# cvlab-yonsei/HVPR

Hardware: AMD Instinct MI355X
Metric: KITTI frames/sec/GPU (fwd, ~20k pts); VFE+scatter achieved HBM GB/s vs peak (higher is better)
Workload: dtype f32; 1 GPU; hvpr_car.yaml batch=1 forward-only, a1..a8 (on-GPU voxelize, pillar VFE, memory read-out + scatter, BEV backbone, head + decode, score top-k + rotated-BEV NMS); frames sharded over ranks, replicas only; global_batch=1, weights=deterministic synthetic (seed 0), BN stats randomised, cls bias -4.595

## Files before the change

hvpr_amd/_lib.py:

```python
import ctypes
import os

_HERE = os.path.dirname(os.path.abspath(__file__))
ABI_VERSION = 8
LIB_PATH = os.environ.get("HVPR_AMD_LIB", os.path.join(_HERE, "libhvpr_amd.so"))

_c = ctypes
_P = _c.c_void_p
_I = _c.c_int
_F = _c.c_float
_Z = _c.c_size_t
ALLREDUCE_FN = _c.CFUNCTYPE(_I, _P, _I, _P, _P)

SIGNATURES = {
    "hvpr_abi_version": (_I, []),
    "hvpr_status_string": (_c.c_char_p, [_I]),
    "hvpr_set_batchnorm_allreduce": (None, [_P, _P]),
    "hvpr_voxelize_workspace_bytes": (_Z, [_I, _I, _I, _I, _I]),
    "hvpr_voxelize_workspace_reset": (_I, [_P, _Z, _I, _I, _I, _I, _I, _P]),
    "hvpr_voxelize_workspace_status": (_I, [_P, _Z, _I, _I, _I, _I, _I, _P]),
    "hvpr_voxelize_f32": (_I, [_P, _I, _I, _I, _I, _P, _I, _F, _F, _F, _F, _F, _F, _I, _I, _I, _I, _I, _I,
                               _P, _P, _P, _P, _I, _P, _Z, _I, _I, _P]),
    "hvpr_pillar_vfe_fwd_f32": (_I, [_P, _P, _P, _I, _I, _P, _F, _F, _F, _F, _F, _F, _P, _P, _P, _P, _P, _P, _P, _P,
                                     _P, _P, _P, _P]),
    "hvpr_memory_bank_packed_floats": (_Z, [_I]),
    "hvpr_memory_bank_pack_f32": (_I, [_P, _I, _P, _P]),
    "hvpr_memory_readout_fwd_f32": (_I, [_P, _I, _P, _P, _P, _I, _I, _P, _P, _P]),
    "hvpr_scatter_workspace_bytes": (_Z, [_I, _I, _I]),
    "hvpr_memory_scatter_fwd_f32": (_I, [_P, _P, _P, _I, _P, _P, _P, _I, _I, _I, _I, _I, _P, _P, _P, _P, _Z, _P]),
    "hvpr_encode_fwd_f32": (_I, [_P, _I, _I, _I, _I, _P, _I, _F, _F, _F, _F, _F, _F, _I, _I, _I, _I, _I, _I, _F, _F, _F,
                                 _P, _P, _P, _P, _P, _P, _P, _P, _P, _P, _I, _I, _P, _P, _P, _P, _I, _P, _P, _P, _P, _P, _P,
                                 _P, _P, _Z, _I, _I, _I, _P]),
    "hvpr_scatter_bev_fwd_f32": (_I, [_P, _I, _P, _I, _P, _I, _P, _I, _P, _I, _I, _I, _P, _P, _P, _Z, _P]),
    "hvpr_spatial_gate_f32": (_I, [_P, _I, _I, _I, _I, _P, _F, _F, _F, _P, _P]),
    "hvpr_head_decode_f32": (_I, [_P, _I, _I, _I, _I, _I, _I, _I, _P, _P, _P, _F, _F, _F, _P, _P, _P, _P, _P]),
    "hvpr_score_topk_workspace_bytes": (_Z, [_I, _I]),
    "hvpr_score_topk_f32": (_I, [_P, _I, _I, _F, _I, _I, _P, _P, _P, _P, _Z, _P]),
    "hvpr_nms_workspace_bytes": (_Z, [_I]),
    "hvpr_nms_bev_f32": (_I, [_P, _I, _P, _P, _I, _F, _I, _I, _P, _P, _P, _Z, _P]),
    "hvpr_gather_predictions_f32": (_I, [_P, _I, _P, _P, _P, _I, _P, _P, _P, _P, _P]),
    "hvpr_boxes_pairwise_f32": (_I, [_P, _I, _P, _I, _I, _P, _P]),
    "hvpr_boxes_pairwise_ragged_f32": (_I, [_P, _P, _P, _P, _P, _I, _c.c_longlong, _P, _P]),
    "hvpr_kitti_overlaps_f64": (_I, [_P, _P, _P, _P, _P, _P, _I, _c.c_longlong, _I, _P, _P]),
    "hvpr_kitti_match_workspace_bytes": (_Z, [_I, _I, _I, _I]),
    "hvpr_kitti_match_f64": (_I, [_P, _P, _P, _P, _P, _P, _P, _P, _I, _c.c_longlong, _P, _I, _I, _P, _I, _P, _I, _P, _P, _I, _I,
                                  _P, _P, _P, _P, _P, _Z, _P]),
    "hvpr_recall_record_f32": (_I, [_P, _P, _I, _I, _P, _I, _I, _P, _I, _P, _P, _P]),
    "hvpr_prediction_annos_f32": (_I, [_P, _P, _P, _P, _I, _I, _P, _P, _I, _P, _c.c_longlong, _I, _I, _P, _P, _P, _P, _P, _P, _P, _P]),
    "hvpr_nms_bev_batched_workspace_bytes": (_Z, [_I, _I]),
    "hvpr_nms_bev_batched_f32": (_I, [_P, _I, _c.c_longlong, _I, _P, _P, _I, _I, _F, _I, _I, _P, _P, _P, _Z, _P]),
    "hvpr_gather_predictions_batched_f32": (_I, [_P, _I, _c.c_longlong, _I, _P, _P, _c.c_longlong, _P, _I, _I, _P, _P, _P, _P, _P]),
    "hvpr_gather_predictions_multiclass_f32": (_I, [_P, _I, _c.c_longlong, _P, _c.c_longlong, _P, _P, _I, _I, _I, _P, _P, _P, _P, _P, _P]),
    "hvpr_furthest_point_sample_f32": (_I, [_P, _I, _I, _I, _P, _P]),
    "hvpr_ball_query_f32": (_I, [_P, _P, _I, _I, _I, _F, _I, _P, _P]),
    "hvpr_three_nn_f32": (_I, [_P, _P, _I, _I, _I, _P, _P, _P]),
    "hvpr_group_points_f32": (_I, [_P, _P, _I, _I, _I, _I, _I, _P, _P]),
    "hvpr_three_interpolate_f32": (_I, [_P, _P, _P, _I, _I, _I, _I, _P, _P]),
    "hvpr_group_rows_f32": (_I, [_P, _P, _P, _P, _I, _I, _I, _I, _I, _I, _P, _P]),
    "hvpr_max_samples_f32": (_I, [_P, _c.c_longlong, _I, _I, _P, _P, _P]),
    "hvpr_max_samples_grad_f32": (_I, [_P, _P, _c.c_longlong, _I, _I, _P, _P]),
    "hvpr_fp_rows_f32": (_I, [_P, _P, _P, _P, _I, _I, _I, _I, _I, _I, _P, _P]),
    "hvpr_spatial_gate_train_workspace_bytes": (_Z, [_I, _I, _I]),
    "hvpr_spatial_gate_train_fwd_f32": (_I, [_P, _I, _I, _I, _I, _P, _P, _P, _P, _F, _P, _P, _P, _P, _P, _P, _Z, _P]),
    "hvpr_spatial_gate_train_bwd_f32": (_I, [_P, _P, _P, _P, _P, _P, _P, _P, _I, _I, _I, _I, _P, _P, _P, _P, _P, _P, _Z, _P]),
    "hvpr_conv2d_wgrad_workspace_bytes": (_Z, [_I, _I, _I, _I, _I, _I, _I]),
    "hvpr_conv2d_wgrad_nhwc_f32": (_I, [_P, _I, _I, _I, _I, _P, _I, _I, _I, _P, _P, _Z, _P]),
    "hvpr_bn_workspace_bytes": (_Z, [_c.c_longlong, _I]),
    "hvpr_bn_stats_nhwc_f32": (_I, [_P, _c.c_longlong, _I, _F, _P, _P, _P, _P, _Z, _P]),
    "hvpr_bn_relu_fwd_nhwc_f32": (_I, [_P, _c.c_longlong, _I, _P, _P, _I, _P, _P, _P, _I, _I, _P]),
    "hvpr_bn_relu_bwd_sums_nhwc_f32": (_I, [_P, _I, _I, _P, _c.c_longlong, _I, _P, _P, _P, _P, _I, _P, _P, _P, _P, _Z, _P]),
    "hvpr_bn_relu_bwd_apply_nhwc_f32": (_I, [_P, _I, _I, _P, _c.c_longlong, _I, _P, _P, _P, _P, _I, _P, _P, _P, _P, _P, _c.c_double, _P]),
    "hvpr_memory_train_workspace_bytes": (_Z, [_I]),
    "hvpr_memory_train_fwd_f32": (_I, [_P, _c.c_longlong, _P, _I, _F, _P, _P, _P, _Z, _P]),
    "hvpr_memory_train_bwd_f32": (_I, [_P, _P, _c.c_longlong, _P, _I, _F, _P, _P, _P, _P, _P, _Z, _P]),
    "hvpr_point_pillar_topk_f32": (_I, [_P, _I, _P, _P, _I, _I, _P, _P]),
    "hvpr_segment_sum_rows_f32": (_I, [_P, _c.c_longlong, _I, _I, _P, _P, _P, _c.c_longlong, _P, _c.c_longlong, _P]),
    "hvpr_attend_rows_fwd_f32": (_I, [_P, _I, _P, _c.c_longlong, _P, _I, _I, _P, _P, _P]),
    "hvpr_fused_adam_truewd_f32": (_I, [_P, _P, _P, _P, _c.c_longlong, _F, _F, _F, _F, _F, _I, _P, _P]),
    "hvpr_fused_adam_l2_f32": (_I, [_P, _P, _P, _P, _c.c_longlong, _F, _F, _F, _F, _F, _I, _P, _P]),
    "hvpr_fused_sgd_f32": (_I, [_P, _P, _P, _c.c_longlong, _F, _F, _F, _P, _P]),
    "hvpr_assign_targets_workspace_bytes": (_Z, [_I, _I]),
    "hvpr_assign_targets_f32": (_I, [_P, _I, _P, _I, _I, _I, _I, _F, _F, _I, _I, _I, _c.c_longlong, _P, _P, _P, _P, _P, _Z, _P]),
    "hvpr_rpn_losses_workspace_bytes": (_Z, [_I, _c.c_longlong]),
    "hvpr_rpn_losses_f32": (_I, [_P, _P, _P, _P, _P, _P, _P, _I, _c.c_longlong, _I, _I, _F, _F, _F, _P, _F, _F, _F, _F, _P, _P, _P, _P,
                                 _P, _Z, _P]),
    "hvpr_mse_loss_workspace_bytes": (_Z, []),
    "hvpr_mse_loss_f32": (_I, [_P, _P, _c.c_longlong, _I, _F, _P, _P, _P, _Z, _P]),
    "hvpr_split_bf16_f32": (_I, [_P, _c.c_longlong, _I, _P, _P]),
    "hvpr_unsplit_bf16_f32": (_I, [_P, _c.c_longlong, _I, _P, _P]),
    "hvpr_conv2d_nhwc_bf16x3": (_I, [_P, _I, _I, _I, _I, _P, _P, _I, _I, _I, _I, _P, _P, _I, _P, _I, _I, _I, _I, _I, _P]),
    "hvpr_deconv_nhwc_bf16x3": (_I, [_P, _I, _I, _I, _I, _P, _P, _I, _I, _I, _I, _P, _I, _I, _I, _P]),
    "hvpr_point_flags_f32": (_I, [_P, _I, _I, _I, _P, _F, _P, _P, _I, _I, _P, _P]),
    "hvpr_compact_workspace_bytes": (_Z, [_I]),
    "hvpr_compact_rows_f32": (_I, [_P, _I, _I, _P, _P, _I, _P, _P, _Z, _P]),
    "hvpr_frame_offsets_f32": (_I, [_P, _I, _I, _I, _P, _P]),
    "hvpr_gather_rows_f32": (_I, [_P, _I, _I, _P, _I, _P, _P]),
    "hvpr_pillar_vfe_train_workspace_bytes": (_Z, []),
    "hvpr_pillar_vfe_train_fwd_f32": (_I, [_P, _P, _P, _I, _I, _P, _P, _P, _P, _P, _P, _F, _F, _F, _F, _F, _F, _F, _P, _P, _P, _P, _P, _P, _Z, _P]),
    "hvpr_pillar_vfe_bwd_f32": (_I, [_P, _P, _P, _I, _I, _P, _P, _P, _P, _P, _P, _F, _F, _F, _F, _F, _F, _F, _P, _P, _P, _P, _P, _P, _P, _P, _Z, _P]),
    "hvpr_conv2d_wino_wgrad_workspace_bytes": (_Z, [_I, _I, _I, _I, _I]),
    "hvpr_conv2d_wino_wgrad_nhwc_f32": (_I, [_P, _I, _I, _I, _I, _P, _I, _P, _P, _Z, _P]),
    "hvpr_conv2d_wino_packed_floats": (_Z, [_I, _I]),
    "hvpr_conv2d_wino_pack_f32": (_I, [_P, _P, _I, _I, _I, _P, _P]),
    "hvpr_conv2d_wino_nhwc_f32": (_I, [_P, _I, _I, _I, _I, _P, _P, _I, _I, _P, _P, _I, _P, _I, _I, _I, _P, _P]),
    "hvpr_conv2d_wino_stats_rows": (_I, [_I, _I, _I]),
    "hvpr_conv2d_wino_items": (_I, [_I, _I, _I, _I, _I]),
    "hvpr_conv2d_wino_tab_bytes": (_Z, [_I, _I, _I, _I, _I]),
    "hvpr_conv2d_wino_tab_build": (_I, [_I, _I, _I, _I, _I, _P, _P]),
    "hvpr_conv2d_wino_nhwc_tab_f32": (_I, [_P, _I, _I, _I, _I, _P, _P, _I, _I, _P, _P, _I, _P, _I, _I, _I, _P, _P, _P]),
    "hvpr_conv2d_tab_bytes": (_Z, [_I, _I, _I, _I, _I, _I, _I]),
    "hvpr_conv2d_tab_build": (_I, [_I, _I, _I, _I, _I, _I, _I, _P, _P]),
    "hvpr_conv2d_nhwc_tab_f32": (_I, [_P, _I, _I, _I, _I, _P, _P, _I, _I, _I, _I, _I, _I, _P, _P, _I, _P, _I, _I, _I, _P, _P]),
    "hvpr_conv2d_s2_dgrad_nhwc_f32": (_I, [_P, _I, _I, _I, _I, _P, _P, _I, _I, _I, _I, _P, _I, _I, _P]),
    "hvpr_bn_train_affine_f32": (_I, [_P, _P, _P, _I, _P, _P, _F, _F, _P, _P, _P, _P, _P, _P]),
    "hvpr_bn_finalize_partials_f32": (_I, [_P, _I, _I, _c.c_longlong, _F, _P, _P, _P, _P]),
    "hvpr_conv2d_nhwc_f32": (_I, [_P, _I, _I, _I, _I, _P, _P, _I, _I, _I, _I, _I, _I, _P, _P, _I, _P, _I, _I, _I, _P]),
    "hvpr_augment_block_points": (_I, []),
    "hvpr_augment_collide_f32": (_I, [_P, _P, _I, _P, _P]),
    "hvpr_augment_boxes_f32": (_I, [_P, _P, _I, _P, _P, _I, _I, _P, _P, _P]),
    "hvpr_augment_points_workspace_bytes": (_Z, [_I, _I, _I, _c.c_longlong]),
    "hvpr_augment_points_f32": (_I, [_P, _P, _I, _P, _P, _c.c_longlong, _I, _P, _c.c_longlong, _P, _I, _I, _P, _P, _c.c_longlong, _P,
                                     _P, _Z, _P]),
    "hvpr_gt_database_block_points": (_I, []),
    "hvpr_gt_database_workspace_bytes": (_Z, [_I, _I, _I]),
    "hvpr_gt_database_count_f32": (_I, [_P, _c.c_longlong, _I, _P, _P, _I, _P, _P, _P, _I, _P, _P, _Z, _P]),
    "hvpr_gt_database_extract_f32": (_I, [_P, _c.c_longlong, _I, _P, _P, _I, _P, _P, _P, _P, _I, _P, _P, _P, _P, _c.c_longlong,
                                          _P, _Z, _P]),
    "hvpr_ragged_select_tile_rows": (_I, []),
    "hvpr_ragged_select_workspace_bytes": (_Z, [_c.c_longlong, _I]),
    "hvpr_ragged_select_count_f32": (_I, [_P, _c.c_longlong, _I, _P, _I, _I, _P, _P, _P, _P, _Z, _P]),
    "hvpr_ragged_select_write_f32": (_I, [_P, _c.c_longlong, _I, _P, _I, _I, _P, _P, _P, _P, _c.c_longlong, _I, _P, _c.c_longlong,
                                          _P, _P, _Z, _P]),
    "hvpr_ragged_sample_workspace_bytes": (_Z, [_c.c_longlong, _I]),
    "hvpr_ragged_sample_count_f32": (_I, [_P, _c.c_longlong, _I, _P, _I, _I, _P, _P, _F, _P, _P, _P, _Z, _P]),
    "hvpr_ragged_sample_write_f32": (_I, [_P, _c.c_longlong, _I, _P, _I, _I, _P, _P, _F, _P, _P, _P, _P, _c.c_longlong, _I, _I, _P,
                                          _c.c_longlong, _P, _P, _Z, _P]),
    "hvpr_kitti_infos_block_points": (_I, []),
    "hvpr_kitti_infos_workspace_bytes": (_Z, [_I, _I, _I]),
    "hvpr_kitti_infos_count_f32": (_I, [_P, _c.c_longlong, _I, _P, _P, _I, _P, _P, _P, _I, _P, _P, _P, _P, _P, _Z, _P]),
    "hvpr_render_bev_workspace_bytes": (_Z, [_I, _I, _I]),
    "hvpr_render_bev_u8": (_I, [_P, _c.c_longlong, _I, _I, _P, _I, _P, _F, _P, _I, _I, _P, _P, _F, _P, _I, _P, _I, _I, _P, _P, _F, _P, _I,
                                _P, _I, _I, _I, _P, _P, _P, _Z, _P]),
}

_lib = None


class HvprLibraryError(RuntimeError):
    pass


def lib():
    global _lib
    if _lib is None:
        if not os.path.exists(LIB_PATH):
            raise HvprLibraryError(
                f"{LIB_PATH} is missing: build it with `python -m hvpr_amd.build` (hipcc --offload-arch=gfx950). "
                "hvpr_amd has no CPU fallback.")
        try:
            L = ctypes.CDLL(LIB_PATH)
        except OSError as e:
            raise HvprLibraryError(f"cannot load {LIB_PATH}: {e}") from e
        for name, (res, args) in SIGNATURES.items():
            fn = getattr(L, name)
            fn.restype = res
            fn.argtypes = args
        if L.hvpr_abi_version() != ABI_VERSION:
            raise HvprLibraryError(f"{LIB_PATH} has ABI version {L.hvpr_abi_version()}, these wrappers need {ABI_VERSION}: "
                                   "rebuild it with `python -m hvpr_amd.build`")
        _lib = L
    return _lib


def check(status, what):
    if status != 0:
        msg = lib().hvpr_status_string(int(status))
        raise RuntimeError(f"{what} failed: {msg.decode() if msg else status}")
```

hvpr_amd/anchor_head.py:

```python
import os

import numpy as np
import torch
import torch.nn as nn

from . import kernels
from .folding import FoldCache


class ResidualCoder:

    def __init__(self, code_size=7, encode_angle_by_sincos=False, **kwargs):
        assert not encode_angle_by_sincos, "HIP decode: plain angle residual"
        self.code_size = code_size
        self.encode_angle_by_sincos = False

    @staticmethod
    def encode_torch(boxes, anchors):
        anchors[:, 3:6] = torch.clamp_min(anchors[:, 3:6], min=1e-5)
        boxes[:, 3:6] = torch.clamp_min(boxes[:, 3:6], min=1e-5)
        xa, ya, za, dxa, dya, dza, ra, *cas = torch.split(anchors, 1, dim=-1)
        xg, yg, zg, dxg, dyg, dzg, rg, *cgs = torch.split(boxes, 1, dim=-1)
        diag = torch.sqrt(dxa ** 2 + dya ** 2)
        parts = [(xg - xa) / diag, (yg - ya) / diag, (zg - za) / dza, torch.log(dxg / dxa), torch.log(dyg / dya),
                 torch.log(dzg / dza), rg - ra] + [g - a for g, a in zip(cgs, cas)]
        return torch.cat(parts, dim=-1)

    @staticmethod
    def decode_torch(enc, anchors):
        xa, ya, za, dxa, dya, dza, ra, *cas = torch.split(anchors, 1, dim=-1)
        xt, yt, zt, dxt, dyt, dzt, rt, *cts = torch.split(enc, 1, dim=-1)
        diag = torch.sqrt(dxa ** 2 + dya ** 2)
        parts = [xt * diag + xa, yt * diag + ya, zt * dza + za, torch.exp(dxt) * dxa, torch.exp(dyt) * dya,
                 torch.exp(dzt) * dza, rt + ra] + [t + a for t, a in zip(cts, cas)]
        return torch.cat(parts, dim=-1)


class AnchorGenerator:

    def __init__(self, anchor_range, anchor_generator_config):
        self.anchor_range = np.asarray(anchor_range, dtype=np.float32)
        self.cfg = anchor_generator_config
        self.anchor_sizes = [c["anchor_sizes"] for c in anchor_generator_config]
        self.anchor_rotations = [c["anchor_rotations"] for c in anchor_generator_config]
        self.anchor_heights = [c["anchor_bottom_heights"] for c in anchor_generator_config]
        self.align_center = [c.get("align_center", False) for c in anchor_generator_config]
        self.num_of_anchor_sets = len(self.anchor_sizes)

    def shifts(self, grid_size, align_center):
        r = self.anchor_range
        gx, gy = np.int64(grid_size[0]), np.int64(grid_size[1])
        if align_center:
            xs, ys = (r[3] - r[0]) / gx, (r[4] - r[1]) / gy
            xo, yo = xs / 2, ys / 2
        else:
            xs, ys = (r[3] - r[0]) / (gx - 1), (r[4] - r[1]) / (gy - 1)
            xo, yo = 0, 0
        x = torch.arange(r[0] + xo, r[3] + 1e-5, step=xs, dtype=torch.float32)
        y = torch.arange(r[1] + yo, r[4] + 1e-5, step=ys, dtype=torch.float32)
        return x, y

    def generate_anchors(self, grid_sizes):
        assert len(grid_sizes) == self.num_of_anchor_sets
        all_anchors, per_loc = [], []
        for gs, sizes, rots, heights, ac in zip(grid_sizes, self.anchor_sizes, self.anchor_rotations, self.anchor_heights,
                                                self.align_center):
            per_loc.append(len(rots) * len(sizes) * len(heights))
            x, y = self.shifts(gs, ac)
            z = torch.tensor(heights, dtype=torch.float32)
            sz = torch.tensor(sizes, dtype=torch.float32)
            rt = torch.tensor(rots, dtype=torch.float32)
            a = torch.zeros(len(z), len(y), len(x), sz.shape[0], rt.shape[0], 7)
            a[..., 0] = x.view(1, 1, -1, 1, 1)
            a[..., 1] = y.view(1, -1, 1, 1, 1)
            a[..., 2] = z.view(-1, 1, 1, 1, 1)
            a[..., 3:6] = sz.view(1, 1, 1, -1, 1, 3)
            a[..., 6] = rt.view(1, 1, 1, 1, -1)
            a[..., 2] += a[..., 5] / 2
            all_anchors.append(a)
        return all_anchors, per_loc


class AnchorHeadTemplate(nn.Module):

    def __init__(self, model_cfg, num_class, class_names, grid_size, point_cloud_range, predict_boxes_when_training):
        super().__init__()
        self.model_cfg = model_cfg
        self.num_class = num_class
        self.class_names = class_names
        self.predict_boxes_when_training = predict_boxes_when_training
        self.use_multihead = model_cfg.get("USE_MULTIHEAD", False)
        assert not self.use_multihead, "hvpr path: single head"
        tcfg = model_cfg.TARGET_ASSIGNER_CONFIG
        assert tcfg.BOX_CODER == "ResidualCoder"
        self.box_coder = ResidualCoder(num_dir_bins=tcfg.get("NUM_DIR_BINS", 6), **tcfg.get("BOX_CODER_CONFIG", {}))
        agc = model_cfg.ANCHOR_GENERATOR_CONFIG
        grid_size = np.asarray(grid_size)
        self.anchor_generator = AnchorGenerator(point_cloud_range, agc)
        self.feature_map_sizes = [grid_size[:2] // c["feature_map_stride"] for c in agc]
        anchors, self.num_anchors_per_location = self.anchor_generator.generate_anchors(self.feature_map_sizes)
        dev = torch.device("cuda") if torch.cuda.is_available() else torch.device("cpu")
        self.anchors = [a.to(dev) for a in anchors]
        self.target_assigner = None
        self.forward_ret_dict = {}

    def _decode_tables(self, device):
        fms = self.feature_map_sizes[0]
        assert all((f == fms).all() for f in self.feature_map_sizes), "single head: one feature-map size"
        x, y = self.anchor_generator.shifts(fms, self.anchor_generator.align_center[0])
        rows = []
        for sizes, rots, heights in zip(self.anchor_generator.anchor_sizes, self.anchor_generator.anchor_rotations,
                                        self.anchor_generator.anchor_heights):
            assert len(heights) == 1
            for s in sizes:
                for r in rots:
                    zc = torch.tensor(heights[0], dtype=torch.float32) + torch.tensor(s[2], dtype=torch.float32) / 2
                    rows.append([float(zc), s[0], s[1], s[2], r])
        return x.to(device), y.to(device), torch.tensor(rows, dtype=torch.float32, device=device)

    def assign_targets(self, gt_boxes):
        if self.target_assigner is None:
            from .target_assigner import AxisAlignedTargetAssigner
            assert self.model_cfg.TARGET_ASSIGNER_CONFIG.NAME == "AxisAlignedTargetAssigner"
            self.target_assigner = AxisAlignedTargetAssigner(self.model_cfg, self.class_names, self.box_coder,
                                                             self.model_cfg.TARGET_ASSIGNER_CONFIG.MATCH_HEIGHT)
        return self.target_assigner.assign_targets([a.to(gt_boxes.device) for a in self.anchors], gt_boxes)

    def _anchor_rot(self, device):
        if getattr(self, "_rot_cache", None) is None or self._rot_cache.device != device:
            self._rot_cache = torch.cat(self.anchors, dim=-3)[..., 6].reshape(-1).to(device=device, dtype=torch.float32).contiguous()
        return self._rot_cache

    def get_loss(self):
        from . import losses
        fr = self.forward_ret_dict
        w = self.model_cfg.LOSS_CONFIG.LOSS_WEIGHTS
        common = dict(labels=fr["box_cls_labels"], reg_targets=fr["box_reg_targets"], anchor_rot=self._anchor_rot(fr["box_preds"].device),
                      pos_count=fr["positives_per_frame"], num_class=self.num_class, cfg_weights=w, dir_offset=self.model_cfg.DIR_OFFSET,
                      num_dir_bins=self.model_cfg.NUM_DIR_BINS)
        cls, box, parts = losses.rpn_losses(fr["cls_preds"], fr["box_preds"], fr.get("dir_cls_preds"), **common)
        cls_p, box_p, parts_p = losses.rpn_losses(fr["cls_preds_point"], fr["box_preds_point"], fr.get("dir_cls_preds_point"), **common)
        mem = losses.memory_loss(fr["pos_memory_feas"], fr["pos_point_feas"], w["mem_weight"])
        tb = {"rpn_loss_cls": parts["cls"], "rpn_loss_loc": parts["loc"], "rpn_loss_cls_pt": parts_p["cls"],
              "rpn_loss_loc_pt": parts_p["loc"], "mem_loss": mem, "rpn_loss": cls + box, "rpn_loss_point": cls_p + box_p}
        if "dir" in parts:
            tb["rpn_loss_dir"], tb["rpn_loss_dir_pt"] = parts["dir"], parts_p["dir"]
        return cls + box, cls_p + box_p, mem, {k: v.detach() for k, v in tb.items()}, fr["memory_items"]

    def generate_predicted_boxes(self, batch_size, cls_preds, box_preds, dir_cls_preds=None):
        from .common_utils import limit_period
        anchors = torch.cat(self.anchors, dim=-3)
        A = anchors.view(-1, anchors.shape[-1]).shape[0]
        batch_anchors = anchors.view(1, -1, anchors.shape[-1]).repeat(batch_size, 1, 1).to(box_preds.device)
        batch_cls = cls_preds.reshape(batch_size, A, -1).float()
        boxes = self.box_coder.decode_torch(box_preds.reshape(batch_size, A, -1), batch_anchors)
        if dir_cls_preds is not None:
            labels = torch.max(dir_cls_preds.reshape(batch_size, A, -1), dim=-1)[1]
            period = 2 * np.pi / self.model_cfg.NUM_DIR_BINS
            rot = limit_period(boxes[..., 6] - self.model_cfg.DIR_OFFSET, self.model_cfg.DIR_LIMIT_OFFSET, period)
            boxes[..., 6] = rot + self.model_cfg.DIR_OFFSET + period * labels.to(boxes.dtype)
        return batch_cls, boxes


class AnchorHeadSingle(AnchorHeadTemplate):

    def __init__(self, model_cfg, input_channels, num_class, class_names, grid_size, point_cloud_range,
                 predict_boxes_when_training=True):
        super().__init__(model_cfg=model_cfg, num_class=num_class, class_names=class_names, grid_size=grid_size,
                         point_cloud_range=point_cloud_range, predict_boxes_when_training=predict_boxes_when_training)
        self.num_anchors_per_location = sum(self.num_anchors_per_location)
        na = self.num_anchors_per_location
        self.conv_cls = nn.Conv2d(input_channels, na * self.num_class, kernel_size=1)
        self.conv_box = nn.Conv2d(input_channels, na * self.box_coder.code_size, kernel_size=1)
        self.num_dir_bins = model_cfg.NUM_DIR_BINS if model_cfg.get("USE_DIRECTION_CLASSIFIER", None) is not None else 0
        self.conv_dir_cls = nn.Conv2d(input_channels, na * self.num_dir_bins, kernel_size=1) if self.num_dir_bins else None
        self.init_weights()
        self._fold = FoldCache()

    def init_weights(self):
        pi = 0.01
        nn.init.constant_(self.conv_cls.bias, -np.log((1 - pi) / pi))
        nn.init.normal_(self.conv_box.weight, mean=0, std=0.001)

    def train(self, mode=True):
        self._fold.invalidate()
        return super().train(mode)

    def _load_from_state_dict(self, *a, **k):
        self._fold.invalidate()
        return super()._load_from_state_dict(*a, **k)

    def _build_packed(self, device):
        convs = [self.conv_cls, self.conv_box] + ([self.conv_dir_cls] if self.conv_dir_cls is not None else [])
        w = torch.cat([c.weight.detach().float() for c in convs], dim=0)
        b = torch.cat([c.bias.detach().float() for c in convs], dim=0)
        x, y, table = self._decode_tables(device)
        return {"pc": kernels.pack_conv(w, None, b, relu=False, tile_cfg=1), "xs": x, "ys": y, "table": table}

    def _forward_train(self, data_dict):
        from . import conv_train as ct
        fr = self.forward_ret_dict
        heads = [self.conv_cls, self.conv_box] + ([self.conv_dir_cls] if self.conv_dir_cls is not None else [])
        f0 = data_dict["spatial_features_2d"]
        if not f0.is_cuda or f0.dtype != torch.float32:
            raise RuntimeError("hvpr_amd: AnchorHeadSingle's training forward needs fp32 GPU tensors (the HIP path has no CPU fallback)")
        w = torch.cat([h.weight for h in heads], dim=0)
        b = torch.cat([h.bias for h in heads], dim=0)
        n_out = w.shape[0]
        pad = (-n_out) % 8
        if pad:
            w = torch.cat([w, w.new_zeros((pad,) + tuple(w.shape[1:]))], dim=0)
        cuts = np.cumsum([0] + [h.weight.shape[0] for h in heads])
        for key, suffix in (("spatial_features_2d", ""), ("spatial_features_point_2d", "_point")):
            out = ct.conv(data_dict[key].permute(0, 2, 3, 1), w)[..., :n_out] + b
            parts = [out[..., cuts[i]:cuts[i + 1]].contiguous() for i in range(len(heads))]
            fr["cls_preds" + suffix], fr["box_preds" + suffix] = parts[0], parts[1]
            if self.conv_dir_cls is not None:
                fr["dir_cls_preds" + suffix] = parts[2]
        return self._finish_train(data_dict)

    def _finish_train(self, data_dict):
        fr = self.forward_ret_dict
        fr["pos_point_feas"] = data_dict["point_positive_features"]
        fr["pos_memory_feas"] = data_dict["memory_positive_features"]
        fr["memory_items"] = data_dict["memory_items"]
        fr.update(self.assign_targets(gt_boxes=data_dict["gt_boxes"]))
        if self.predict_boxes_when_training:
            data_dict["batch_cls_preds"], data_dict["batch_box_preds"] = self.generate_predicted_boxes(
                data_dict["batch_size"], fr["cls_preds"], fr["box_preds"], fr.get("dir_cls_preds"))
            data_dict["cls_preds_normalized"] = False
        return data_dict

    def forward(self, data_dict):
        if self.training:
            return self._forward_train(data_dict)
        f2d = data_dict["spatial_features_2d"]
        x = f2d.permute(0, 2, 3, 1).contiguous()
        P = self._fold.get(x.device, lambda: self._build_packed(x.device))
        head = kernels.conv2d_nhwc(x, P["pc"], use_table=True)
        na, nc, nb = self.num_anchors_per_location, self.num_class, self.num_dir_bins
        self.forward_ret_dict["cls_preds"] = head[..., : na * nc]
        self.forward_ret_dict["box_preds"] = head[..., na * nc: na * (nc + 7)]
        if nb:
            self.forward_ret_dict["dir_cls_preds"] = head[..., na * (nc + 7):]
        period = 2 * np.pi / nb if nb else 1.0
        cls, box, scores, labels = kernels.head_decode(head, na, nc, nb, P["xs"], P["ys"], P["table"],
                                                       self.model_cfg.DIR_OFFSET, self.model_cfg.DIR_LIMIT_OFFSET, period,
                                                       out=data_dict.get("_out_head"))
        data_dict["batch_cls_preds"] = cls
        data_dict["batch_box_preds"] = box
        data_dict["cls_preds_normalized"] = False
        data_dict["batch_max_scores"] = scores
        data_dict["batch_max_labels"] = labels
        return data_dict


__all__ = {
    "AnchorHeadTemplate": AnchorHeadTemplate,
    "AnchorHeadSingle": AnchorHeadSingle,
}
```

hvpr_amd/csrc/conv_igemm.hip:

```cpp
#include <type_traits>

#include "common.h"

namespace {

typedef float f32x16 __attribute__((ext_vector_type(16)));
constexpr int KC = 8;

__device__ __forceinline__ void lds_dma16(const void *sbase_uniform, unsigned voff_bytes, unsigned lds_dst_uniform) {
    unsigned keep;
    asm volatile("s_mov_b32 %0, m0\n\ts_mov_b32 m0, %3\n\ts_nop 0\n\tglobal_load_lds_dwordx4 %1, %2\n\ts_mov_b32 m0, %0"
                 : "=&s"(keep)
                 : "v"(voff_bytes), "s"(sbase_uniform), "s"(lds_dst_uniform)
                 : "memory");
}

__device__ __forceinline__ unsigned lds_addr_of(const void *p) {
    return (unsigned)(size_t)(const __attribute__((address_space(3))) void *)p;
}

struct ConvArgs {
    const float *in;
    const float *wpk;
    const float *bias;
    float *out;
    const float *gate;
    const float *resid;
    int N, H, W, Cin;
    int OH, OW;
    int cout_gemm;
    int cout_pad;
    int out_cstride, out_coff, resid_cstride;
    int relu;
    int up;
    int cout_real;
    int tiles_x, tiles_y, n_ct;
    const unsigned long long *tab;
};

enum { OPT_TAB = 1, OPT_PEEL = 2 };
#ifndef HVPR_ITEM_OPT
#define HVPR_ITEM_OPT (OPT_TAB | OPT_PEEL)
#endif

constexpr int TAB_MAX_TX = 1 << 16, TAB_MAX_TY = 1 << 15, TAB_MAX_CT = 1 << 12, TAB_MAX_N = 1 << 20;
__device__ __forceinline__ unsigned long long tab_load(const unsigned long long *tab, int step) {
    return *((const __attribute__((address_space(4))) unsigned long long *)(size_t)tab + step);
}

#ifdef HVPR_EXP_TIMING
__device__ long long g_conv_dbg[8 * 4 * 64 * 4];
#endif

template <int TH, int TW, int BN, int S, int TAPS, bool UP2 = false, int OPT = 0>
__global__ void __launch_bounds__(256) k_conv(ConvArgs a) {
    static_assert(!UP2 || (TAPS == 9 && S == 1 && TH == 16 && TW == 16), "UP2: 16 x 16 output tiles of a 3x3 stride-2 layer's data gradient");
    static_assert(!UP2 || OPT == 0, "the item switches belong to the forward instantiations");
    constexpr bool TAB = (OPT & OPT_TAB) != 0, PEEL = (OPT & OPT_PEEL) != 0;
    constexpr int BM = TH * TW;
    constexpr int WM = BM / 2, WN = BN / 2;
    constexpr int MB = WM / 32, NB = WN / 32;
    static_assert(MB >= 1 && NB >= 1, "wave tile must hold at least one 32x32 block");
    constexpr int HALO = TAPS == 9 ? 2 : 0;
    constexpr int NSUB = TAPS == 4 ? 4 : 1;
    constexpr int KSTAGE = KC * NSUB;
    constexpr int PH = UP2 ? TH / 2 + 1 : (TH - 1) * S + 1 + HALO, PW = UP2 ? TW / 2 + 1 : (TW - 1) * S + 1 + HALO;
    constexpr int PPAD = (PH * PW + 63) / 64 * 64;
    constexpr int PATCH_V4 = NSUB * 2 * PPAD;
    constexpr int W_V4 = TAPS * BN * 2;
    constexpr int NLD_P = (PATCH_V4 + 255) / 256, NLD_W = (W_V4 + 255) / 256;

    constexpr int PATCH_PAD = NLD_P * 256, W_PAD = NLD_W * 256;
    __shared__ __attribute__((aligned(16))) float4 s_patch[2][PATCH_PAD];
    __shared__ __attribute__((aligned(16))) float4 s_w[2][W_PAD];
    __shared__ __attribute__((aligned(16))) float4 s_bias[BN / 4];

    const int tid = threadIdx.x, lane = tid & 63, wid = tid >> 6;
    const unsigned wave_s = __builtin_amdgcn_readfirstlane((unsigned)(threadIdx.x >> 6));
    const int wm = wid >> 1, wn = wid & 1;
    const int half = lane >> 5, l31 = lane & 31;

    int p_py[NLD_P], p_px[NLD_P], p_part[NLD_P];
    bool p_live[NLD_P];
#pragma unroll
    for (int i = 0; i < NLD_P; ++i) {
        const int v = tid + i * 256;
        const int part = v / PPAD, pix = v % PPAD;
        p_py[i] = pix / PW; p_px[i] = pix % PW; p_part[i] = part * 4;
        p_live[i] = v < PATCH_V4 && pix < PH * PW;
    }
    unsigned woff0[NLD_W];
    bool wok[NLD_W];
    const size_t w_chunk_stride = (size_t)a.cout_pad * KC;
    const size_t w_tap_stride = (size_t)(a.Cin / KC) * w_chunk_stride;
#pragma unroll
    for (int i = 0; i < NLD_W; ++i) {
        const int v = tid + i * 256;
        wok[i] = v < W_V4;
        const int th = v / BN, co_l = v % BN;
        const int tap = th >> 1, hf = th & 1;
        const size_t tap_stride = TAPS == 4 ? w_chunk_stride : w_tap_stride;
        woff0[i] = wok[i] ? (unsigned)(((size_t)tap * tap_stride + ((size_t)hf * a.cout_pad + co_l) * 4) * sizeof(float)) : 0u;
    }
    int a_off[MB];
#pragma unroll
    for (int mb = 0; mb < MB; ++mb) {
        const int q = mb * 32 + l31;
        const int py = wm * (TH / 2) + q / TW, px = q % TW;
        a_off[mb] = half * PPAD + (py * S) * PW + px * S;
        if (UP2) a_off[mb] = half * PPAD + (wm * 4 + (l31 >> 3)) * PW + (l31 & 7);
    }
    int b_off[NB];
#pragma unroll
    for (int nb = 0; nb < NB; ++nb) b_off[nb] = half * BN + wn * WN + nb * 32 + l31;
    const unsigned lds_patch0 = lds_addr_of(&s_patch[0][0]) + wave_s * 1024u;
    const unsigned lds_w0 = lds_addr_of(&s_w[0][0]) + wave_s * 1024u;

    const int n_pt = a.tiles_x * a.tiles_y * a.N;
    const int total_walk = ((n_pt + 7) / 8) * 8 * a.n_ct;
#ifdef HVPR_EXP_TIMING
    int dbg_tile = 0;
    const int dbg_slot = (blockIdx.x % 97 == 5 && blockIdx.x / 97 < 8) ? (int)(blockIdx.x / 97) : -1;
#endif
    unsigned long long e_next = 0ull;
    if (TAB && (int)blockIdx.x < total_walk) e_next = tab_load(a.tab, blockIdx.x);
    for (int it = blockIdx.x; it < total_walk; it += gridDim.x) {
    int ct, tx, ty, n;
    if constexpr (TAB) {
        const unsigned lo = (unsigned)e_next, hi = (unsigned)(e_next >> 32);
        if (it + (int)gridDim.x < total_walk) e_next = tab_load(a.tab, it + (int)gridDim.x);
        if (lo >> 31) continue;
        tx = (int)(lo & 0xffffu); ty = (int)(lo >> 16 & 0x7fffu); ct = (int)(hi & 0xfffu); n = (int)(hi >> 12);
        if (n >= a.N || ct >= a.n_ct) continue;
    } else {
        const int xcd = it & 7, j = it >> 3;
        ct = j % a.n_ct;
        int pt = (j / a.n_ct) * 8 + xcd;
        if (pt >= n_pt) continue;
        tx = pt % a.tiles_x; pt /= a.tiles_x;
        ty = pt % a.tiles_y;
        n = pt / a.tiles_y;
    }
    const int oy0 = ty * TH, ox0 = tx * TW;
    const int iy0 = UP2 ? oy0 / 2 : oy0 * S - (HALO / 2), ix0 = UP2 ? ox0 / 2 : ox0 * S - (HALO / 2);
    const int co0 = ct * BN;

    unsigned poff[NLD_P];
    bool pok[NLD_P];
#pragma unroll
    for (int i = 0; i < NLD_P; ++i) {
        const int iy = iy0 + p_py[i], ix = ix0 + p_px[i];
        pok[i] = p_live[i] && iy >= 0 && iy < a.H && ix >= 0 && ix < a.W;
        poff[i] = pok[i] ? (unsigned)(((iy * a.W + ix) * a.Cin + p_part[i]) * (int)sizeof(float)) : 0u;
    }
    const unsigned w_co0 = (unsigned)(co0 * 4 * sizeof(float));
    const char *in_n = (const char *)(a.in + (size_t)n * a.H * a.W * a.Cin);

    auto stage_piece = [&](int chunk, int buf, int i) {
        if (i < NLD_P) {
            const char *pbase = in_n + (size_t)chunk * (KSTAGE * sizeof(float));
            if (pok[i]) lds_dma16(pbase, poff[i], lds_patch0 + (unsigned)(buf * PATCH_PAD + i * 256) * 16u);
        } else {
            const int j = i - NLD_P;
            const char *wbase = (const char *)a.wpk + (size_t)chunk * NSUB * w_chunk_stride * sizeof(float);
            if (wok[j]) lds_dma16(wbase, woff0[j] + w_co0, lds_w0 + (unsigned)(buf * W_PAD + j * 256) * 16u);
        }
    };
    auto stage = [&](int chunk, int buf) {
#pragma unroll
        for (int i = 0; i < NLD_P + NLD_W; ++i) stage_piece(chunk, buf, i);
    };
    constexpr int DEAL = TAPS == 9 ? 6 : (TAPS == 4 ? 3 : 0);
    const bool border = iy0 < 0 || ix0 < 0 || iy0 + PH > a.H || ix0 + PW > a.W;
    if (border) {
#pragma unroll
        for (int b = 0; b < 2; ++b)
#pragma unroll
            for (int i = 0; i < NLD_P; ++i) s_patch[b][tid + i * 256] = make_float4(0.f, 0.f, 0.f, 0.f);
        __syncthreads();
    }
    if (tid < BN / 4) s_bias[tid] = *(const float4 *)(a.bias + co0 + tid * 4);
    f32x16 acc[MB][NB];
    if (!PEEL) {
#pragma unroll
        for (int mb = 0; mb < MB; ++mb)
#pragma unroll
            for (int nb = 0; nb < NB; ++nb)
#pragma unroll
                for (int r = 0; r < 16; ++r) acc[mb][nb][r] = 0.f;
    }

    const int n_chunks = a.Cin / KSTAGE;
    auto chunk_step = [&](int c, auto buf_tag, auto first_tag) {
        constexpr int BUF = decltype(buf_tag)::value;
        constexpr bool FIRST = decltype(first_tag)::value;
#ifdef HVPR_EXP_TIMING
        const long long q0 = __builtin_readcyclecounter();
#endif
        asm volatile("s_waitcnt vmcnt(0)" ::: "memory");
        __builtin_amdgcn_s_barrier();
#ifdef HVPR_EXP_TIMING
        const long long q1 = __builtin_readcyclecounter();
#endif
        if (DEAL == 0 && c + 1 < n_chunks) stage(c + 1, BUF ^ 1);
#ifdef HVPR_EXP_TIMING
        const long long q2 = __builtin_readcyclecounter();
#endif
        const float4 *sp = s_patch[BUF];
        const float4 *sw = s_w[BUF];
        constexpr int PF = TAPS >= 3 ? 2 : 0;
        float4 av[PF + 1][MB], bv[PF + 1][NB];
        auto up2_uses = [](int mb, int tap) { return (((mb >> 1) == 0) == (tap / 3 == 1)) && (((mb & 1) == 0) == (tap % 3 == 1)); };
        auto lds_load = [&](int tap, int slot) {
            const int ky = TAPS == 9 ? tap / 3 : 0, kx = TAPS == 9 ? tap % 3 : 0;
#pragma unroll
            for (int mb = 0; mb < MB; ++mb) {
                if (UP2) {
                    if (up2_uses(mb, tap)) av[slot][mb] = sp[a_off[mb] + (ky == 0 ? PW : 0) + (kx == 0 ? 1 : 0)];
                    continue;
                }
                av[slot][mb] = sp[a_off[mb] + (TAPS == 4 ? tap * 2 * PPAD : ky * PW + kx)];
            }
#pragma unroll
            for (int nb = 0; nb < NB; ++nb) bv[slot][nb] = sw[b_off[nb] + tap * BN * 2];
        };
#pragma unroll
        for (int t = 0; t < PF; ++t) lds_load(t, t);
#pragma unroll
        for (int tap = 0; tap < TAPS; ++tap) {
            if (tap + PF < TAPS || PF == 0) lds_load(tap + PF < TAPS ? tap + PF : tap, (tap + PF) % (PF + 1));
            __builtin_amdgcn_sched_barrier(0);
            const int cur = tap % (PF + 1);
#pragma unroll
            for (int mb = 0; mb < MB; ++mb)
#pragma unroll
                for (int nb = 0; nb < NB; ++nb) {
                    if (UP2 && !up2_uses(mb, tap)) continue;
                    if (PEEL && FIRST && tap == 0) acc[mb][nb] = __builtin_amdgcn_mfma_f32_32x32x2f32(bv[cur][nb].x, av[cur][mb].x, f32x16{}, 0, 0, 0);
                    else acc[mb][nb] = __builtin_amdgcn_mfma_f32_32x32x2f32(bv[cur][nb].x, av[cur][mb].x, acc[mb][nb], 0, 0, 0);
                    acc[mb][nb] = __builtin_amdgcn_mfma_f32_32x32x2f32(bv[cur][nb].y, av[cur][mb].y, acc[mb][nb], 0, 0, 0);
                    acc[mb][nb] = __builtin_amdgcn_mfma_f32_32x32x2f32(bv[cur][nb].z, av[cur][mb].z, acc[mb][nb], 0, 0, 0);
                    acc[mb][nb] = __builtin_amdgcn_mfma_f32_32x32x2f32(bv[cur][nb].w, av[cur][mb].w, acc[mb][nb], 0, 0, 0);
                }
            __builtin_amdgcn_sched_barrier(0);
            if (DEAL > 0 && tap < DEAL && c + 1 < n_chunks) {
                constexpr int NPC = (NLD_P + NLD_W + DEAL - 1) / (DEAL > 0 ? DEAL : 1);
#pragma unroll
                for (int i = tap * NPC; i < (tap + 1) * NPC && i < NLD_P + NLD_W; ++i) stage_piece(c + 1, BUF ^ 1, i);
                __builtin_amdgcn_sched_barrier(0);
            }
        }
#ifdef HVPR_EXP_TIMING
        if (dbg_slot >= 0 && dbg_tile == 1 && c < 64) {
            asm volatile("" ::"v"(acc[0][0][0]));
            long long *d = g_conv_dbg + (((size_t)dbg_slot * 4 + wid) * 64 + c) * 4;
            d[0] = q0; d[1] = q1; d[2] = q2; d[3] = __builtin_readcyclecounter();
        }
#endif
    };
    stage(0, 0);
    if constexpr (PEEL) {
        chunk_step(0, std::integral_constant<int, 0>{}, std::true_type{});
        for (int c = 1; c + 1 < n_chunks; c += 2) {
            chunk_step(c, std::integral_constant<int, 1>{}, std::false_type{});
            chunk_step(c + 1, std::integral_constant<int, 0>{}, std::false_type{});
        }
        if (!(n_chunks & 1)) chunk_step(n_chunks - 1, std::integral_constant<int, 1>{}, std::false_type{});
    } else {
        for (int c = 0; c + 1 < n_chunks; c += 2) {
            chunk_step(c, std::integral_constant<int, 0>{}, std::false_type{});
            chunk_step(c + 1, std::integral_constant<int, 1>{}, std::false_type{});
        }
        if (n_chunks & 1) chunk_step(n_chunks - 1, std::integral_constant<int, 0>{}, std::false_type{});
    }

#pragma unroll
    for (int mb = 0; mb < MB; ++mb) {
        const int q = mb * 32 + l31;
        const int oy = UP2 ? oy0 + 2 * (wm * 4 + (l31 >> 3)) + (mb >> 1) : oy0 + wm * (TH / 2) + q / TW;
        const int ox = UP2 ? ox0 + 2 * (l31 & 7) + (mb & 1) : ox0 + q % TW;
        if (oy >= a.OH || ox >= a.OW) continue;
        const size_t pix = ((size_t)n * a.OH + oy) * a.OW + ox;
        const float gate = a.gate ? a.gate[pix] : 0.f;
        const float *rrow = a.gate ? a.resid + pix * a.resid_cstride : nullptr;
#pragma unroll
        for (int nb = 0; nb < NB; ++nb) {
#pragma unroll
            for (int g = 0; g < 4; ++g) {
                const int col = co0 + wn * WN + nb * 32 + 8 * g + 4 * half;
                if (col >= a.cout_gemm) continue;
                const float4 bias = s_bias[(col - co0) >> 2];
                float4 y = make_float4(acc[mb][nb][4 * g] + bias.x, acc[mb][nb][4 * g + 1] + bias.y,
                                       acc[mb][nb][4 * g + 2] + bias.z, acc[mb][nb][4 * g + 3] + bias.w);
                if (a.relu) { y.x = fmaxf(y.x, 0.f); y.y = fmaxf(y.y, 0.f); y.z = fmaxf(y.z, 0.f); y.w = fmaxf(y.w, 0.f); }
                int co = col, sy = 0, sx = 0;
                if (a.up > 1) { const int sub = col / a.cout_real; co = col - sub * a.cout_real; sy = sub / a.up; sx = sub % a.up; }
                if (a.gate) {
                    const float4 r = *(const float4 *)(rrow + co);
                    y.x = fmaf(gate, y.x, r.x); y.y = fmaf(gate, y.y, r.y); y.z = fmaf(gate, y.z, r.z); y.w = fmaf(gate, y.w, r.w);
                }
                const size_t opix = a.up > 1 ? ((size_t)n * a.OH * a.up + (oy * a.up + sy)) * ((size_t)a.OW * a.up) + (ox * a.up + sx) : pix;
                *(float4 *)(a.out + opix * a.out_cstride + a.out_coff + co) = y;
            }
        }
    }
    __syncthreads();
#ifdef HVPR_EXP_TIMING
    ++dbg_tile;
#endif
    }
}

__global__ void k_conv_tab(int N, int tiles_x, int tiles_y, int n_ct, int total_walk, unsigned long long *__restrict__ tab) {
    const int it = blockIdx.x * blockDim.x + threadIdx.x;
    if (it >= total_walk) return;
    const int xcd = it & 7, j = it >> 3;
    const int ct = j % n_ct;
    int pt = (j / n_ct) * 8 + xcd;
    if (pt >= tiles_x * tiles_y * N) {
        tab[it] = 1ull << 31;
        return;
    }
    const int tx = pt % tiles_x; pt /= tiles_x;
    const int ty = pt % tiles_y;
    const int n = pt / tiles_y;
    tab[it] = (unsigned long long)((unsigned)tx | (unsigned)ty << 16) | (unsigned long long)((unsigned)ct | (unsigned)n << 12) << 32;
}

static int conv_tab_grid(int N, int H, int W, int taps, int stride, int cout_pad, int tile_cfg, int &tiles_x, int &tiles_y, int &n_ct) {
    if (N < 1 || H < 1 || W < 1 || cout_pad < 1 || (taps != 9 && taps != 1) || (stride != 1 && stride != 2) || tile_cfg < 0 || tile_cfg > 2) return 0;
    const int OH = taps == 9 ? (H + 2 - 3) / stride + 1 : H, OW = taps == 9 ? (W + 2 - 3) / stride + 1 : W;
    const int tw = tile_cfg == 1 ? 8 : 16, bn = tile_cfg == 0 ? 128 : 64;
    if (OH < 1 || OW < 1 || cout_pad % bn != 0) return 0;
    tiles_x = (OW + tw - 1) / tw; tiles_y = (OH + 7) / 8; n_ct = cout_pad / bn;
    if (tiles_x > TAB_MAX_TX || tiles_y > TAB_MAX_TY || n_ct > TAB_MAX_CT || N > TAB_MAX_N) return 0;
    const long long steps = ((long long)N * tiles_x * tiles_y + 7) / 8 * 8 * n_ct;
    return steps < (1ll << 28) ? (int)steps : 0;
}

template <int TH, int TW, int BN, int S, int TAPS, bool UP2 = false, int OPT = 0>
int launch(ConvArgs a, hipStream_t s) {
    a.tiles_x = (a.OW + TW - 1) / TW;
    a.tiles_y = (a.OH + TH - 1) / TH;
    a.n_ct = a.cout_pad / BN;
    const long long tiles = (long long)a.N * a.tiles_x * a.tiles_y * a.n_ct;
    static int resident = 0;
    if (resident == 0) {
        int per_cu = 0, dev = 0, cus = 256;
        hipDeviceProp_t prop;
        if (hipGetDevice(&dev) == hipSuccess && hipGetDeviceProperties(&prop, dev) == hipSuccess) cus = prop.multiProcessorCount;
        if (hipOccupancyMaxActiveBlocksPerMultiprocessor(&per_cu, k_conv<TH, TW, BN, S, TAPS, UP2, OPT>, 256, 0) != hipSuccess || per_cu < 1)
            per_cu = 1;
        resident = per_cu * cus;
    }
    long long blocks = tiles < resident ? (tiles + 7) / 8 * 8 : resident;
    if (blocks > resident && resident >= 8) blocks = resident / 8 * 8;
    hipLaunchKernelGGL((k_conv<TH, TW, BN, S, TAPS, UP2, OPT>), dim3((unsigned)blocks), dim3(256), 0, s, a);
    return 0;
}

}

#ifdef HVPR_EXP_TIMING
extern "C" int hvpr_exp_conv_dbg(long long *host_out, int n_words) {
    return hipMemcpyFromSymbol(host_out, HIP_SYMBOL(g_conv_dbg), sizeof(long long) * n_words) == hipSuccess ? 0 : -1;
}
#endif

extern "C" int hvpr_conv2d_s2_dgrad_nhwc_f32(const float *dz, int N, int H, int W, int Cin, const float *w_packed, const float *bias, int cout,
                                             int cout_pad, int OH, int OW, float *dx, int out_cstride, int out_coff, hvpr_stream_t stream) {
    if (!dz || !w_packed || !bias || !dx || N < 1 || H < 1 || W < 1 || Cin < 8 || cout < 1 || OH < 1 || OW < 1) return HVPR_ERR_INVALID_ARG;
    if (H != (OH + 2 - 3) / 2 + 1 || W != (OW + 2 - 3) / 2 + 1) return HVPR_ERR_INVALID_ARG;
    if (Cin % KC != 0 || cout % 4 != 0 || out_cstride % 4 != 0 || out_coff % 4 != 0 || cout_pad % 64 != 0 || cout_pad < cout) return HVPR_ERR_UNSUPPORTED;
    if ((long long)H * W * Cin * 4 >= (1ll << 31)) return HVPR_ERR_UNSUPPORTED;
    ConvArgs a;
    a.in = dz; a.wpk = w_packed; a.bias = bias; a.out = dx; a.gate = nullptr; a.resid = nullptr;
    a.N = N; a.H = H; a.W = W; a.Cin = Cin;
    a.OH = OH; a.OW = OW;
    a.cout_gemm = cout; a.cout_pad = cout_pad; a.cout_real = cout;
    a.out_cstride = out_cstride; a.out_coff = out_coff; a.resid_cstride = 0;
    a.relu = 0; a.up = 1; a.tab = nullptr;
    launch<16, 16, 64, 1, 9, true>(a, (hipStream_t)stream);
    HVPR_CHECK_LAUNCH();
    return HVPR_OK;
}

extern "C" size_t hvpr_conv2d_tab_bytes(int N, int H, int W, int taps, int stride, int cout_pad, int tile_cfg) {
    int tiles_x, tiles_y, n_ct;
    return (size_t)conv_tab_grid(N, H, W, taps, stride, cout_pad, tile_cfg, tiles_x, tiles_y, n_ct) * sizeof(unsigned long long);
}

extern "C" int hvpr_conv2d_tab_build(int N, int H, int W, int taps, int stride, int cout_pad, int tile_cfg, void *table, hvpr_stream_t stream) {
    if (!table) return HVPR_ERR_INVALID_ARG;
    int tiles_x, tiles_y, n_ct;
    const int steps = conv_tab_grid(N, H, W, taps, stride, cout_pad, tile_cfg, tiles_x, tiles_y, n_ct);
    if (steps == 0) return HVPR_ERR_UNSUPPORTED;
    hipLaunchKernelGGL(k_conv_tab, dim3(hvpr_cdiv(steps, 256)), dim3(256), 0, (hipStream_t)stream, N, tiles_x, tiles_y, n_ct, steps,
                       (unsigned long long *)table);
    HVPR_CHECK_LAUNCH();
    return HVPR_OK;
}

static int conv_nhwc(const float *in, int N, int H, int W, int Cin, const float *w_packed,
                     const float *bias, int taps, int stride, int cout, int cout_pad, int up,
                     int relu, const float *gate, const float *resid, int resid_cstride, float *out,
                     int out_cstride, int out_coff, int tile_cfg, const void *table, hvpr_stream_t stream) {
    if (!in || !w_packed || !bias || !out || N < 1 || H < 1 || W < 1 || Cin < 8 || cout < 1) return HVPR_ERR_INVALID_ARG;
    if ((gate == nullptr) != (resid == nullptr)) return HVPR_ERR_INVALID_ARG;
    if (Cin % KC != 0 || (taps != 9 && taps != 1) || (stride != 1 && stride != 2) || up < 1) return HVPR_ERR_UNSUPPORTED;
    const bool wide1x1 = taps == 1 && Cin % (4 * KC) == 0;
    if (taps == 1 && stride != 1) return HVPR_ERR_UNSUPPORTED;
    if (up > 1 && (taps != 1 || gate)) return HVPR_ERR_UNSUPPORTED;
    if (cout % 4 != 0 || out_cstride % 4 != 0 || out_coff % 4 != 0 || (resid && resid_cstride % 4 != 0)) return HVPR_ERR_UNSUPPORTED;
    if ((long long)H * W * Cin * 4 >= (1ll << 31)) return HVPR_ERR_UNSUPPORTED;
    ConvArgs a;
    a.in = in; a.wpk = w_packed; a.bias = bias; a.out = out; a.gate = gate; a.resid = resid;
    a.N = N; a.H = H; a.W = W; a.Cin = Cin;
    a.OH = taps == 9 ? (H + 2 - 3) / stride + 1 : H;
    a.OW = taps == 9 ? (W + 2 - 3) / stride + 1 : W;
    a.cout_gemm = up > 1 ? cout * up * up : cout;
    a.cout_pad = cout_pad; a.cout_real = cout;
    a.out_cstride = out_cstride; a.out_coff = out_coff; a.resid_cstride = resid_cstride;
    a.relu = relu; a.up = up;
    a.tab = (HVPR_ITEM_OPT & OPT_TAB) ? (const unsigned long long *)table : nullptr;
    if (cout_pad < a.cout_gemm) return HVPR_ERR_INVALID_ARG;
    if (table && hvpr_conv2d_tab_bytes(N, H, W, taps, stride, cout_pad, tile_cfg) == 0) return HVPR_ERR_UNSUPPORTED;
    hipStream_t s = (hipStream_t)stream;
    const int bn = tile_cfg == 0 ? 128 : 64;
    if (cout_pad % bn != 0) return HVPR_ERR_INVALID_ARG;
    constexpr int OPT0 = HVPR_ITEM_OPT & ~OPT_TAB;
#define HV_CASE(TH, TW, BN, OPT)                                                    \
    if (taps == 9 && stride == 1) launch<TH, TW, BN, 1, 9, false, OPT>(a, s);       \
    else if (taps == 9 && stride == 2) launch<TH, TW, BN, 2, 9, false, OPT>(a, s);  \
    else if (wide1x1) launch<TH, TW, BN, 1, 4, false, OPT>(a, s);                   \
    else launch<TH, TW, BN, 1, 1, false, OPT>(a, s);
#define HV_TILE(TH, TW, BN)                                                         \
    if (a.tab) { HV_CASE(TH, TW, BN, OPT0 | OPT_TAB) } else { HV_CASE(TH, TW, BN, OPT0) }
    if (tile_cfg == 0) { HV_TILE(8, 16, 128) }
    else if (tile_cfg == 1) { HV_TILE(8, 8, 64) }
    else if (tile_cfg == 2) { HV_TILE(8, 16, 64) }
    else return HVPR_ERR_INVALID_ARG;
#undef HV_TILE
#undef HV_CASE
    HVPR_CHECK_LAUNCH();
    return HVPR_OK;
}

extern "C" int hvpr_conv2d_nhwc_f32(const float *in, int N, int H, int W, int Cin, const float *w_packed,
                                    const float *bias, int taps, int stride, int cout, int cout_pad, int up,
                                    int relu, const float *gate, const float *resid, int resid_cstride, float *out,
                                    int out_cstride, int out_coff, int tile_cfg, hvpr_stream_t stream) {
    return conv_nhwc(in, N, H, W, Cin, w_packed, bias, taps, stride, cout, cout_pad, up, relu, gate, resid, resid_cstride, out, out_cstride,
                     out_coff, tile_cfg, nullptr, stream);
}

extern "C" int hvpr_conv2d_nhwc_tab_f32(const float *in, int N, int H, int W, int Cin, const float *w_packed,
                                        const float *bias, int taps, int stride, int cout, int cout_pad, int up,
                                        int relu, const float *gate, const float *resid, int resid_cstride, float *out,
                                        int out_cstride, int out_coff, int tile_cfg, const void *table, hvpr_stream_t stream) {
    return conv_nhwc(in, N, H, W, Cin, w_packed, bias, taps, stride, cout, cout_pad, up, relu, gate, resid, resid_cstride, out, out_cstride,
                     out_coff, tile_cfg, table, stream);
}
```

hvpr_amd/kernels.py:

```python
import os

import torch

from ._lib import check, lib


def _stream():
    return torch.cuda.current_stream().cuda_stream


def _ptr(t, dtype=None, name="tensor"):
    if t is None:
        return None
    if not t.is_cuda:
        raise RuntimeError(f"hvpr_amd: {name} must live on the GPU (the HIP path has no CPU fallback)")
    if dtype is not None and t.dtype != dtype:
        raise TypeError(f"hvpr_amd: {name} must be {dtype}, got {t.dtype}")
    if not t.is_contiguous():
        raise ValueError(f"hvpr_amd: {name} must be contiguous")
    return t.data_ptr()


class VoxelizeWorkspace:

    def __init__(self, batch, n_points, grid, device):
        self.key = (int(batch), int(n_points), tuple(int(g) for g in grid), torch.device(device))
        nx, ny, nz = self.key[2]
        nbytes = lib().hvpr_voxelize_workspace_bytes(batch, n_points, nx, ny, nz)
        self.buf = torch.empty(nbytes, dtype=torch.uint8, device=device)
        self.reset()

    def reset(self):
        batch, n_points, (nx, ny, nz), _ = self.key
        check(lib().hvpr_voxelize_workspace_reset(self.buf.data_ptr(), self.buf.numel(), batch, n_points, nx, ny, nz,
                                                  _stream()), "hvpr_voxelize_workspace_reset")

    def status(self):
        batch, n_points, (nx, ny, nz), _ = self.key
        check(lib().hvpr_voxelize_workspace_status(self.buf.data_ptr(), self.buf.numel(), batch, n_points, nx, ny, nz,
                                                   _stream()), "hvpr_voxelize_workspace_status")


def voxelize(points, frame_offsets, batch, point_cloud_range, voxel_size, grid, max_points, max_voxels, workspace,
             xyz_col=0, n_feat=None, cap_mode=0, capacity=None):
    n, stride = points.shape
    n_feat = stride - xyz_col if n_feat is None else n_feat
    if capacity is None:
        capacity = min(n, batch * max_voxels)
    dev = points.device
    voxels = torch.empty((capacity, max_points, n_feat), dtype=torch.float32, device=dev)
    coords = torch.empty((capacity, 4), dtype=torch.int32, device=dev)
    num = torch.empty((capacity,), dtype=torch.int32, device=dev)
    offs = torch.empty((batch + 1,), dtype=torch.int32, device=dev)
    nx, ny, nz = [int(g) for g in grid]
    lo = [float(torch.tensor(v, dtype=torch.float32)) for v in point_cloud_range[:3]]
    vs = [float(torch.tensor(v, dtype=torch.float32)) for v in voxel_size]
    if workspace.key[0] < batch or workspace.key[1] < n:
        raise ValueError("voxelize workspace too small for this call")
    check(lib().hvpr_voxelize_f32(_ptr(points, torch.float32, "points"), n, stride, xyz_col, n_feat,
                                  _ptr(frame_offsets, torch.int32, "frame_offsets"), batch, lo[0], lo[1], lo[2],
                                  vs[0], vs[1], vs[2], nx, ny, nz, int(max_points), int(max_voxels), int(cap_mode),
                                  voxels.data_ptr(), coords.data_ptr(), num.data_ptr(), offs.data_ptr(), capacity,
                                  workspace.buf.data_ptr(), workspace.buf.numel(), workspace.key[0], workspace.key[1],
                                  _stream()), "hvpr_voxelize_f32")
    return voxels, coords, num, offs


def pillar_vfe_fwd(voxels, num_points, coords, folded, voxel_size, offsets, m_device=None, want_mask=True):
    M, P, C = voxels.shape
    if C != 4:
        raise ValueError("hvpr_pillar_vfe_fwd_f32 is built for 4 raw point features")
    dev = voxels.device
    pf = torch.empty((M, 64), dtype=torch.float32, device=dev)
    sf = torch.empty((M, 32), dtype=torch.float32, device=dev)
    mask = torch.empty((M, P, 1), dtype=torch.float32, device=dev) if want_mask else None
    check(lib().hvpr_pillar_vfe_fwd_f32(
        _ptr(voxels, torch.float32, "voxels"), _ptr(num_points, torch.int32, "voxel_num_points"),
        _ptr(coords, torch.int32, "voxel_coords"), M, P, _ptr(m_device, torch.int32, "m_device"),
        float(voxel_size[0]), float(voxel_size[1]), float(voxel_size[2]), float(offsets[0]), float(offsets[1]),
        float(offsets[2]), _ptr(folded["w0"], torch.float32), _ptr(folded["b0"], torch.float32),
        _ptr(folded["w1"], torch.float32), _ptr(folded["b1"], torch.float32), _ptr(folded["ws0"], torch.float32),
        _ptr(folded["bs0"], torch.float32), _ptr(folded["ws1"], torch.float32), _ptr(folded["bs1"], torch.float32),
        pf.data_ptr(), sf.data_ptr(), _ptr(mask), _stream()), "hvpr_pillar_vfe_fwd_f32")
    return pf, sf, mask


class PackedBank:

    def __init__(self, weight):
        w = weight.detach().float().contiguous()
        if w.dim() != 2 or w.shape[1] != 64:
            raise ValueError("PackedBank: (n_items, 64) memory bank expected")
        self.n_items = int(w.shape[0])
        self.shape = w.shape
        self.rows = w
        self.data = torch.empty(lib().hvpr_memory_bank_packed_floats(self.n_items), dtype=torch.float32, device=w.device)
        check(lib().hvpr_memory_bank_pack_f32(_ptr(w, torch.float32, "memory.weight"), self.n_items, self.data.data_ptr(), _stream()),
              "hvpr_memory_bank_pack_f32")


def _bank_args(bank):
    if not isinstance(bank, PackedBank):
        _ptr(bank, torch.float32, "memory.weight")
        bank = PackedBank(bank)
    return bank.rows.data_ptr(), bank.data.data_ptr(), bank.n_items


def memory_readout_fwd(f, bank, k, m_device=None, want_idx=False):
    M, C = f.shape
    out = torch.empty((M, C), dtype=torch.float32, device=f.device)
    idx = torch.empty((M, k), dtype=torch.int32, device=f.device) if want_idx else None
    check(lib().hvpr_memory_readout_fwd_f32(_ptr(f, torch.float32, "pillar_features"), M,
                                            _ptr(m_device, torch.int32, "m_device"), *_bank_args(bank), int(k),
                                            out.data_ptr(), _ptr(idx), _stream()), "hvpr_memory_readout_fwd_f32")
    return (out, idx) if want_idx else out


_SEG_CHUNK = 32


def edges_by_destination(dst, n_dst):
    dst = dst.reshape(-1).to(torch.int64)
    dev = dst.device
    E = dst.numel()
    n_max = E // _SEG_CHUNK + min(n_dst, E) + 1
    if E == 0:
        z = torch.zeros(1, dtype=torch.int32, device=dev)
        return torch.zeros(0, dtype=torch.int32, device=dev), z.expand(n_max + 1).contiguous(), z.expand(n_dst + 1).contiguous()
    order = torch.argsort(dst, stable=True)
    sdst = dst[order].contiguous()
    rowptr = torch.searchsorted(sdst, torch.arange(n_dst + 1, dtype=torch.int64, device=dev))
    end_live = rowptr[n_dst:]
    pos = torch.arange(E, dtype=torch.int64, device=dev)
    live = (sdst >= 0) & (sdst < n_dst)
    first = rowptr[sdst.clamp(0, n_dst - 1)]
    head = live & (((pos - first) % _SEG_CHUNK) == 0)
    csum = torch.cumsum(head.to(torch.int64), 0)
    cid, total = csum - 1, csum[-1:]
    chunk_ptr = end_live.expand(n_max + 1).clone()
    chunk_ptr.scatter_(0, torch.where(head, cid, torch.full_like(cid, n_max)), torch.where(head, pos, end_live.expand(E)))
    dest_ptr = torch.where(rowptr < end_live, cid[rowptr.clamp(max=E - 1)], total.expand(n_dst + 1))
    return order.to(torch.int32), chunk_ptr.to(torch.int32), dest_ptr.to(torch.int32)


def segment_sum_rows(src, src_off, C, edge_row, edge_w, chunk_ptr, dest_ptr, n_dst):
    n_chunks = chunk_ptr.numel() - 1
    part = torch.empty((n_chunks, C), dtype=torch.float32, device=src.device)
    check(lib().hvpr_segment_sum_rows_f32(_ptr(src, torch.float32, "src"), src.shape[-1], int(src_off), int(C), _ptr(edge_row, torch.int32, "edge_row"),
                                          _ptr(edge_w, torch.float32, "edge_w"), _ptr(chunk_ptr, torch.int32, "chunk_ptr"), int(n_chunks),
                                          part.data_ptr(), int(C), _stream()), "hvpr_segment_sum_rows_f32")
    dst = torch.empty((n_dst, C), dtype=torch.float32, device=src.device)
    check(lib().hvpr_segment_sum_rows_f32(part.data_ptr(), int(C), 0, int(C), None, None, _ptr(dest_ptr, torch.int32, "dest_ptr"), int(n_dst),
                                          dst.data_ptr(), int(C), _stream()), "hvpr_segment_sum_rows_f32")
    return dst


class EdgePlan:

    def __init__(self, dst, n_dst):
        self.idx, self.n_dst, self._per_batch = dst, int(n_dst), None
        self._plan, self._rows, self._i32 = None, {}, None

    @classmethod
    def batched(cls, idx, n_per_batch):
        plan = cls(idx, idx.shape[0] * int(n_per_batch))
        plan._per_batch = int(n_per_batch)
        return plan

    def build(self):
        if self._plan is None:
            dst = self.idx
            if self._per_batch is not None:
                B = dst.shape[0]
                dst = dst.reshape(B, -1).to(torch.int64) + torch.arange(B, device=dst.device, dtype=torch.int64).view(B, 1) * self._per_batch
            self._plan = edges_by_destination(dst, self.n_dst)
        return self

    def tensors(self):
        made = list(self._plan or ()) + list(self._rows.values())
        return made if self._i32 is None else made + [self._i32]

    def idx32(self):
        if self._i32 is None:
            self._i32 = self.idx.to(torch.int32).contiguous()
        return self._i32

    def edge_rows(self, per=1):
        if per not in self._rows:
            order = self.build()._plan[0]
            self._rows[per] = order if per == 1 else torch.div(order, per, rounding_mode="floor")
        return self._rows[per]

    def edge_weights(self, weights):
        return torch.index_select(weights.reshape(-1), 0, self.build()._plan[0])

    def sum_rows(self, src, src_off=0, C=None, *, per=1, weights=None):
        _, chunk_ptr, dest_ptr = self.build()._plan
        C = src.shape[-1] - src_off if C is None else C
        return segment_sum_rows(src, src_off, C, self.edge_rows(per), None if weights is None else self.edge_weights(weights),
                                chunk_ptr, dest_ptr, self.n_dst)


def attend_rows(q, rows, idx=None, k=None):
    if idx is not None:
        if idx.dim() != 2 or (k is not None and int(k) != idx.shape[1]):
            raise ValueError("hvpr_amd: attend_rows needs idx of shape (M, k)")
        k = idx.shape[1]
    elif k is None:
        raise ValueError("hvpr_amd: attend_rows without idx needs k")
    M, C = q.shape
    if rows.dim() != 2 or rows.shape[1] != C or (idx is not None and idx.shape[0] != M):
        raise ValueError("hvpr_amd: attend_rows needs q (M, C), rows (N, C) and idx (M, k)")
    qp, rp, ip = _ptr(q, torch.float32, "q"), _ptr(rows, torch.float32, "rows"), _ptr(idx, torch.int32, "idx")
    out = torch.empty((M, C), dtype=torch.float32, device=q.device)
    w = torch.empty((M, int(k)), dtype=torch.float32, device=q.device)
    check(lib().hvpr_attend_rows_fwd_f32(qp, M, rp, rows.shape[0], ip, int(k), C, out.data_ptr(), w.data_ptr(), _stream()),
          "hvpr_attend_rows_fwd_f32")
    return out, w


def scatter_workspace(batch, nx, ny, device):
    n = lib().hvpr_scatter_workspace_bytes(batch, nx, ny) // 4
    return torch.full((n,), -1, dtype=torch.int32, device=device)


def scatter_bev_fwd(pillar, memory, scale, coords, batch, nx, ny, workspace, m_device=None):
    M, cp = pillar.shape
    cm = 0 if memory is None else memory.shape[1]
    cs = 0 if scale is None else scale.shape[1]
    dev = pillar.device
    spatial = torch.empty((batch, ny, nx, cp + cm), dtype=torch.float32, device=dev)
    spatial_scale = torch.empty((batch, ny, nx, cs), dtype=torch.float32, device=dev) if cs else None
    check(lib().hvpr_scatter_bev_fwd_f32(_ptr(pillar, torch.float32, "pillar_features"), cp, _ptr(memory, torch.float32),
                                         cm, _ptr(scale, torch.float32), cs, _ptr(coords, torch.int32, "voxel_coords"),
                                         M, _ptr(m_device, torch.int32), batch, nx, ny, spatial.data_ptr(),
                                         _ptr(spatial_scale), workspace.data_ptr(), workspace.numel() * 4, _stream()),
          "hvpr_scatter_bev_fwd_f32")
    spatial = spatial.permute(0, 3, 1, 2)
    if spatial_scale is not None:
        spatial_scale = spatial_scale.permute(0, 3, 1, 2)
    return spatial, spatial_scale


class PackedConvBf3:

    def __init__(self, w, bias, cin, cout, cout_pad, stride, relu, tile_cfg, planes, up=None, out_split=True):
        self.w, self.bias, self.cin, self.cout, self.cout_pad = w, bias, cin, cout, cout_pad
        self.stride, self.relu, self.tile_cfg, self.planes, self.up, self.out_split = stride, relu, tile_cfg, planes, up, out_split

    def fp32_output(self):
        return PackedConvBf3(self.w, self.bias, self.cin, self.cout, self.cout_pad, self.stride, self.relu, self.tile_cfg, self.planes,
                             out_split=False)


def _planes_of(x, planes):
    out, r = [], x
    for _ in range(planes):
        h = r.to(torch.bfloat16)
        out.append(h)
        r = r - h.float()
    return out


def pack_conv_bf3(weight, scale=None, shift=None, stride=1, relu=True, tile_cfg=0, planes=2):
    cout, cin, kh, kw = weight.shape
    assert kh == kw == 3 and cin % 16 == 0 and cout % 4 == 0 and planes in (2, 3)
    w = weight.detach().float()
    if scale is not None:
        w = w * scale.view(-1, 1, 1, 1)
    cout_pad = (cout + 63) // 64 * 64
    wp = torch.zeros((9, cin // 8, planes, cout_pad, 8), dtype=torch.bfloat16, device=w.device)
    for k, part in enumerate(_planes_of(w, planes)):
        wp[:, :, k, :cout, :] = part.permute(2, 3, 1, 0).reshape(9, cin // 8, 8, cout).permute(0, 1, 3, 2)
    b = torch.zeros((cout_pad,), dtype=torch.float32, device=w.device)
    if shift is not None:
        b[:cout] = shift.detach().float()
    return PackedConvBf3(wp.contiguous(), b, cin, cout, cout_pad, stride, relu, tile_cfg, planes)


def pack_deconv_bf3(weight, scale, shift, relu=True, planes=2):
    cin, cout, s, s2 = weight.shape
    assert s == s2 and cin % 64 == 0 and cout % 4 == 0 and planes in (2, 3)
    w = weight.detach().float() * scale.view(1, -1, 1, 1)
    cols = s * s * cout
    cout_pad = (cols + 63) // 64 * 64
    g = w.permute(0, 2, 3, 1).reshape(cin, cols)
    wp = torch.zeros((1, cin // 8, planes, cout_pad, 8), dtype=torch.bfloat16, device=w.device)
    for k, part in enumerate(_planes_of(g, planes)):
        wp[0, :, k, :cols, :] = part.reshape(cin // 8, 8, cols).permute(0, 2, 1)
    b = torch.zeros((cout_pad,), dtype=torch.float32, device=w.device)
    b[:cols] = shift.detach().float().repeat(s * s)
    return PackedConvBf3(wp.contiguous(), b, cin, cout, cout_pad, 1, relu, 1, planes, up=s)


def deconv_nhwc_bf3(xs, pc, out, out_coff=0):
    N, H, W, groups, planes, _ = xs.shape
    assert groups * 8 == pc.cin and planes == pc.planes and xs.is_contiguous()
    assert out.shape[:3] == (N, H * pc.up, W * pc.up) and out.is_contiguous() and out.dtype == torch.float32
    check(lib().hvpr_deconv_nhwc_bf16x3(xs.data_ptr(), N, H, W, pc.cin, pc.w.data_ptr(), pc.bias.data_ptr(), pc.cout, pc.cout_pad,
                                        pc.up, 1 if pc.relu else 0, out.data_ptr(), out.shape[-1], out_coff, planes, _stream()),
          "hvpr_deconv_nhwc_bf16x3")
    return out


def split_bf16(x, planes=2):
    assert x.is_contiguous() and x.shape[-1] % 8 == 0 and x.dtype == torch.float32
    out = torch.empty((*x.shape[:-1], x.shape[-1] // 8, planes, 8), dtype=torch.bfloat16, device=x.device)
    check(lib().hvpr_split_bf16_f32(_ptr(x, torch.float32, "activations"), x.numel(), planes, out.data_ptr(), _stream()),
          "hvpr_split_bf16_f32")
    return out


def unsplit_bf16(xs):
    assert xs.is_contiguous() and xs.dtype == torch.bfloat16 and xs.shape[-1] == 8
    planes = xs.shape[-2]
    out = torch.empty((*xs.shape[:-3], xs.shape[-3] * 8), dtype=torch.float32, device=xs.device)
    check(lib().hvpr_unsplit_bf16_f32(xs.data_ptr(), out.numel(), planes, out.data_ptr(), _stream()), "hvpr_unsplit_bf16_f32")
    return out


def conv2d_nhwc_bf3(xs, pc, out_split=True, gate=None, resid=None):
    N, H, W, groups, planes, _ = xs.shape
    cin = groups * 8
    assert cin == pc.cin and planes == pc.planes and xs.is_contiguous()
    OH, OW = (H + 2 - 3) // pc.stride + 1, (W + 2 - 3) // pc.stride + 1
    if out_split:
        assert pc.cout % 8 == 0
        out = torch.empty((N, OH, OW, pc.cout // 8, planes, 8), dtype=torch.bfloat16, device=xs.device)
    else:
        out = torch.empty((N, OH, OW, pc.cout), dtype=torch.float32, device=xs.device)
    check(lib().hvpr_conv2d_nhwc_bf16x3(xs.data_ptr(), N, H, W, cin, pc.w.data_ptr(), pc.bias.data_ptr(), pc.stride, pc.cout,
                                        pc.cout_pad, 1 if pc.relu else 0, _ptr(gate, torch.float32, "gate"),
                                        None if resid is None else resid.data_ptr(), 0 if resid is None else resid.shape[3] * 8,
                                        out.data_ptr(), 1 if out_split else 0, pc.cout, 0, pc.tile_cfg, planes, _stream()),
          "hvpr_conv2d_nhwc_bf16x3")
    return out


def memory_scatter_fwd(pillar, scale, coords, bank, k, batch, nx, ny, workspace, m_device=None, out=None):
    M = pillar.shape[0]
    dev = pillar.device
    mem = torch.empty((M, 64), dtype=torch.float32, device=dev)
    if out is not None:
        spatial, spatial_scale = (o.permute(0, 2, 3, 1) for o in out)
        if spatial.shape != (batch, ny, nx, 128) or spatial_scale.shape != (batch, ny, nx, 32) or not spatial.is_contiguous() \
                or not spatial_scale.is_contiguous():
            raise ValueError("memory_scatter_fwd: `out` canvases do not match this call")
    else:
        spatial = torch.empty((batch, ny, nx, 128), dtype=torch.float32, device=dev)
        spatial_scale = torch.empty((batch, ny, nx, 32), dtype=torch.float32, device=dev)
    if pillar.shape[1] != 64 or scale.shape[1] != 32 or bank.shape[1] != 64:
        raise ValueError("memory_scatter_fwd is specialised for 64 pillar / 64 memory / 32 scale channels")
    check(lib().hvpr_memory_scatter_fwd_f32(_ptr(pillar, torch.float32, "pillar_features"), _ptr(scale, torch.float32, "scale"),
                                            _ptr(coords, torch.int32, "voxel_coords"), M, _ptr(m_device, torch.int32),
                                            *_bank_args(bank), int(k), batch, nx, ny,
                                            mem.data_ptr(), spatial.data_ptr(), spatial_scale.data_ptr(), workspace.data_ptr(),
                                            workspace.numel() * 4, _stream()), "hvpr_memory_scatter_fwd_f32")
    return mem, spatial.permute(0, 3, 1, 2), spatial_scale.permute(0, 3, 1, 2)


def frame_offsets(points, batch):
    offs = torch.empty((batch + 1,), dtype=torch.int32, device=points.device)
    check(lib().hvpr_frame_offsets_f32(_ptr(points, torch.float32, "points"), points.shape[0], points.shape[1], int(batch),
                                       offs.data_ptr(), _stream()), "hvpr_frame_offsets_f32")
    return offs


def encode_fwd(points, frame_offsets, batch, point_cloud_range, voxel_size, grid, max_points, max_voxels, workspace, folded,
               offsets, bank, k, xyz_col=0, cap_mode=0, capacity=None, want_voxels=True, want_mask=True, out=None, state=None,
               index_mode=0):
    n, stride = points.shape
    n_feat = stride - xyz_col
    if capacity is None:
        capacity = min(n, batch * max_voxels)
    dev = points.device
    nx, ny, nz = [int(g) for g in grid]
    voxels = torch.empty((capacity, max_points, n_feat), dtype=torch.float32, device=dev) if want_voxels else None
    coords = torch.empty((capacity, 4), dtype=torch.int32, device=dev)
    num = torch.empty((capacity,), dtype=torch.int32, device=dev)
    offs = torch.empty((batch + 1,), dtype=torch.int32, device=dev)
    pf = torch.empty((capacity, 64), dtype=torch.float32, device=dev)
    sf = torch.empty((capacity, 32), dtype=torch.float32, device=dev)
    mem = torch.empty((capacity, 64), dtype=torch.float32, device=dev)
    mask = torch.empty((capacity, max_points, 1), dtype=torch.float32, device=dev) if want_mask else None
    if out is not None:
        spatial, spatial_scale = (o.permute(0, 2, 3, 1) for o in out)
        if spatial.shape != (batch, ny, nx, 128) or spatial_scale.shape != (batch, ny, nx, 32) or not spatial.is_contiguous() \
                or not spatial_scale.is_contiguous():
            raise ValueError("encode_fwd: `out` canvases do not match this call")
    else:
        spatial = torch.empty((batch, ny, nx, 128), dtype=torch.float32, device=dev)
        spatial_scale = torch.empty((batch, ny, nx, 32), dtype=torch.float32, device=dev)
    if bank.shape[1] != 64:
        raise ValueError("encode_fwd is specialised for 64 pillar / 64 memory / 32 scale channels")
    if state is not None and (out is None or state.dtype != torch.uint8 or state.numel() != batch * ny * nx or not state.is_contiguous()):
        raise ValueError("encode_fwd: `state` is the (B*ny*nx,) uint8 occupancy of the `out` canvases")
    lo = [float(torch.tensor(v, dtype=torch.float32)) for v in point_cloud_range[:3]]
    vs = [float(torch.tensor(v, dtype=torch.float32)) for v in voxel_size]
    if workspace.key[0] < batch or workspace.key[1] < n:
        raise ValueError("voxelize workspace too small for this call")
    check(lib().hvpr_encode_fwd_f32(
        _ptr(points, torch.float32, "points"), n, stride, xyz_col, n_feat, _ptr(frame_offsets, torch.int32, "frame_offsets"),
        batch, lo[0], lo[1], lo[2], vs[0], vs[1], vs[2], nx, ny, nz, int(max_points), int(max_voxels), int(cap_mode),
        float(offsets[0]), float(offsets[1]), float(offsets[2]),
        _ptr(folded["w0"], torch.float32), _ptr(folded["b0"], torch.float32), _ptr(folded["w1"], torch.float32),
        _ptr(folded["b1"], torch.float32), _ptr(folded["ws0"], torch.float32), _ptr(folded["bs0"], torch.float32),
        _ptr(folded["ws1"], torch.float32), _ptr(folded["bs1"], torch.float32), *_bank_args(bank), int(k), _ptr(voxels), coords.data_ptr(), num.data_ptr(), offs.data_ptr(), capacity, pf.data_ptr(),
        sf.data_ptr(), _ptr(mask), mem.data_ptr(), spatial.data_ptr(), spatial_scale.data_ptr(), _ptr(state), workspace.buf.data_ptr(),
        workspace.buf.numel(), workspace.key[0], workspace.key[1], int(index_mode), _stream()), "hvpr_encode_fwd_f32")
    return {"voxels": voxels, "coords": coords, "num_points": num, "voxel_offsets": offs, "pillar_features": pf,
            "pillar_scale_features": sf, "pillar_mask": mask, "memory_features": mem,
            "spatial": spatial.permute(0, 3, 1, 2), "spatial_scale": spatial_scale.permute(0, 3, 1, 2)}


def canvas_buffers(batch, nx, ny, device):
    sp = torch.zeros((batch, ny, nx, 128), dtype=torch.float32, device=device).permute(0, 3, 1, 2)
    sc = torch.zeros((batch, ny, nx, 32), dtype=torch.float32, device=device).permute(0, 3, 1, 2)
    return (sp, sc), torch.zeros((batch * ny * nx,), dtype=torch.uint8, device=device)


class PackedConv:

    __slots__ = ("w", "bias", "taps", "stride", "cout", "cout_pad", "up", "cin", "relu", "tile_cfg", "tabs")

    def __init__(self, w, bias, taps, stride, cout, cout_pad, up, cin, relu, tile_cfg):
        self.w, self.bias, self.taps, self.stride = w, bias, taps, stride
        self.cout, self.cout_pad, self.up, self.cin, self.relu, self.tile_cfg = cout, cout_pad, up, cin, relu, tile_cfg
        self.tabs = {}


def _tile_channels(tile_cfg):
    return 128 if tile_cfg == 0 else 64


def pack_conv(weight, scale=None, shift=None, stride=1, relu=True, tile_cfg=0):
    cout, cin, kh, kw = weight.shape
    assert kh == kw and kh in (1, 3) and cin % 8 == 0
    w = weight.detach().float()
    if scale is not None:
        w = w * scale.view(-1, 1, 1, 1)
    tc = _tile_channels(tile_cfg)
    cout_pad = (cout + tc - 1) // tc * tc
    taps = kh * kw
    p = w.permute(2, 3, 1, 0).reshape(taps, cin // 8, 2, 4, cout).permute(0, 1, 2, 4, 3)
    wp = torch.zeros((taps, cin // 8, 2, cout_pad, 4), dtype=torch.float32, device=w.device)
    wp[:, :, :, :cout] = p
    b = torch.zeros((cout_pad,), dtype=torch.float32, device=w.device)
    if shift is not None:
        b[:cout] = shift.detach().float()
    return PackedConv(wp.contiguous(), b, taps, stride, cout, cout_pad, 1, cin, relu, tile_cfg)


_zero_bias = {}


class PackedConvWino:

    __slots__ = ("w", "bias", "cout", "cout_pad", "cin", "relu", "px_groups", "tabs")
    taps, stride, up = 9, 1, 1

    def __init__(self, w, bias, cout, cout_pad, cin, relu, px_groups):
        self.w, self.bias, self.cout, self.cout_pad, self.cin, self.relu, self.px_groups = w, bias, cout, cout_pad, cin, relu, px_groups
        self.tabs = {}


def _walk_table(pc, N, H, W, device):
    key = (N, H, W)
    t = pc.tabs.get(key)
    if t is None:
        if torch.cuda.is_current_stream_capturing():
            return 0
        if isinstance(pc, PackedConvWino):
            shape = (N, H, W, pc.cout, pc.px_groups)
            size, build = lib().hvpr_conv2d_wino_tab_bytes, lib().hvpr_conv2d_wino_tab_build
        else:
            shape = (N, H, W, pc.taps, pc.stride, pc.cout_pad, pc.tile_cfg)
            size, build = lib().hvpr_conv2d_tab_bytes, lib().hvpr_conv2d_tab_build
        nbytes = size(*shape)
        t = torch.empty((nbytes // 8,), dtype=torch.int64, device=device)
        if nbytes:
            check(build(*shape, t.data_ptr(), _stream()), "walk table build")
            torch.cuda.current_stream().synchronize()
        pc.tabs[key] = t
    return t.data_ptr() if t.numel() else 0


def pack_conv_wino(weight, scale=None, shift=None, relu=True, px_groups=1, adjoint=False):
    w = weight.detach()
    if w.dtype != torch.float32 or not w.is_contiguous():
        w = w.float().contiguous()
    cout, cin = (w.shape[1], w.shape[0]) if adjoint else (w.shape[0], w.shape[1])
    assert w.shape[2:] == (3, 3) and cin % 8 == 0 and cout % 4 == 0
    cout_pad = (cout + 63) // 64 * 64
    wp = torch.empty((lib().hvpr_conv2d_wino_packed_floats(cin, cout),), dtype=torch.float32, device=w.device)
    sc = None if scale is None else scale.detach().float().contiguous()
    check(lib().hvpr_conv2d_wino_pack_f32(_ptr(w, torch.float32, "conv weight"), _ptr(sc, torch.float32, "scale"), cout, cin,
                                          1 if adjoint else 0, wp.data_ptr(), _stream()), "hvpr_conv2d_wino_pack_f32")
    if shift is None:
        key = (cout_pad, w.device)
        if key not in _zero_bias:
            _zero_bias[key] = torch.zeros((cout_pad,), dtype=torch.float32, device=w.device)
        b = _zero_bias[key]
    else:
        b = torch.zeros((cout_pad,), dtype=torch.float32, device=w.device)
        b[:cout] = shift.detach().float()
    return PackedConvWino(wp, b, cout, cout_pad, cin, relu, px_groups)


def conv2d_wino_nhwc(x, pc, out=None, out_coff=0, gate=None, resid=None, bn_partials=None, use_table=False):
    N, H, W, cin = x.shape
    assert cin == pc.cin
    if out is None:
        out = torch.empty((N, H, W, pc.cout), dtype=torch.float32, device=x.device)
    assert out.shape[:3] == (N, H, W) and out.is_contiguous()
    tab = _walk_table(pc, N, H, W, x.device) if use_table and bn_partials is None and pc.px_groups == 1 else 0
    check(lib().hvpr_conv2d_wino_nhwc_tab_f32(_ptr(x, torch.float32, "conv input"), N, H, W, cin, pc.w.data_ptr(), pc.bias.data_ptr(),
                                              pc.cout, 1 if pc.relu else 0, _ptr(gate, torch.float32, "gate"),
                                              _ptr(resid, torch.float32, "resid"), 0 if resid is None else resid.shape[-1],
                                              out.data_ptr(), out.shape[-1], int(out_coff), pc.px_groups,
                                              _ptr(bn_partials, torch.float32, "bn_partials"), tab, _stream()),
          "hvpr_conv2d_wino_nhwc_tab_f32")
    return out


def pack_deconv(weight, scale, shift, relu=True, tile_cfg=0):
    cin, cout, s, s2 = weight.shape
    assert s == s2 and cin % 8 == 0
    w = weight.detach().float() * scale.view(1, -1, 1, 1)
    cols = s * s * cout
    tc = _tile_channels(tile_cfg)
    cout_pad = (cols + tc - 1) // tc * tc
    g = w.permute(0, 2, 3, 1).reshape(cin, cols)
    p = g.reshape(cin // 8, 2, 4, cols).permute(0, 1, 3, 2).unsqueeze(0)
    wp = torch.zeros((1, cin // 8, 2, cout_pad, 4), dtype=torch.float32, device=w.device)
    wp[:, :, :, :cols] = p
    b = torch.zeros((cout_pad,), dtype=torch.float32, device=w.device)
    b[:cols] = shift.detach().float().repeat(s * s)
    return PackedConv(wp.contiguous(), b, 1, 1, cout, cout_pad, s, cin, relu, tile_cfg)


def conv_algo():
    algo = os.environ.get("HVPR_CONV_ALGO", "winograd")
    if algo not in ("winograd", "direct"):
        raise ValueError(f"HVPR_CONV_ALGO must be 'winograd' or 'direct', got {algo!r}")
    return algo


def pack_conv_auto(weight, scale=None, shift=None, stride=1, relu=True, tile_cfg=1, px_groups=1):
    if weight.shape[2] == 3 and stride == 1 and weight.shape[0] % 4 == 0 and weight.shape[1] % 8 == 0 and conv_algo() == "winograd":
        return pack_conv_wino(weight, scale, shift, relu=relu, px_groups=px_groups)
    return pack_conv(weight, scale, shift, stride=stride, relu=relu, tile_cfg=tile_cfg)


def conv2d_nhwc(x, pc, out=None, out_coff=0, gate=None, resid=None, use_table=False):
    if isinstance(pc, PackedConvBf3):
        if pc.up is not None:
            assert gate is None and resid is None
            return deconv_nhwc_bf3(x, pc, out, out_coff=out_coff)
        assert out is None, "the split-bf16 convolution allocates its own output"
        return conv2d_nhwc_bf3(x, pc, out_split=pc.out_split, gate=gate, resid=resid)
    if x.dtype == torch.bfloat16:
        x = unsplit_bf16(x)
    if isinstance(pc, PackedConvWino):
        return conv2d_wino_nhwc(x, pc, out=out, out_coff=out_coff, gate=gate, resid=resid, use_table=use_table)
    N, H, W, cin = x.shape
    assert cin == pc.cin
    if pc.taps == 9:
        OH, OW = (H + 2 - 3) // pc.stride + 1, (W + 2 - 3) // pc.stride + 1
    else:
        OH, OW = H, W
    if out is None:
        out = torch.empty((N, OH * pc.up, OW * pc.up, pc.cout), dtype=torch.float32, device=x.device)
    assert out.shape[:3] == (N, OH * pc.up, OW * pc.up) and out.is_contiguous()
    tab = _walk_table(pc, N, H, W, x.device) if use_table else 0
    check(lib().hvpr_conv2d_nhwc_tab_f32(_ptr(x, torch.float32, "conv input"), N, H, W, cin, pc.w.data_ptr(),
                                         pc.bias.data_ptr(), pc.taps, pc.stride, pc.cout, pc.cout_pad, pc.up,
                                         1 if pc.relu else 0, _ptr(gate, torch.float32, "gate"),
                                         _ptr(resid, torch.float32, "resid"), 0 if resid is None else resid.shape[-1],
                                         out.data_ptr(), out.shape[-1], int(out_coff), pc.tile_cfg, tab, _stream()),
          "hvpr_conv2d_nhwc_tab_f32")
    return out


def pack_conv_s2_dgrad(weight):
    return pack_conv(weight.detach().permute(1, 0, 2, 3), None, None, stride=1, relu=False, tile_cfg=1)


def conv2d_s2_dgrad_nhwc(dz, weight, H, W, pc=None):
    N, OH, OW, cout = dz.shape
    cin = weight.shape[1]
    assert weight.shape[0] == cout and tuple(weight.shape[2:]) == (3, 3) and OH == (H + 2 - 3) // 2 + 1 and OW == (W + 2 - 3) // 2 + 1
    if pc is None:
        pc = pack_conv_s2_dgrad(weight)
    dx = torch.empty((N, H, W, cin), dtype=torch.float32, device=dz.device)
    check(lib().hvpr_conv2d_s2_dgrad_nhwc_f32(_ptr(dz, torch.float32, "dz"), N, OH, OW, cout, pc.w.data_ptr(), pc.bias.data_ptr(), cin,
                                              pc.cout_pad, H, W, dx.data_ptr(), cin, 0, _stream()), "hvpr_conv2d_s2_dgrad_nhwc_f32")
    return dx


def spatial_gate(y_nhwc, w18, conv_bias, bn_scale, bn_shift):
    N, H, W, C = y_nhwc.shape
    gate = torch.empty((N, H, W), dtype=torch.float32, device=y_nhwc.device)
    check(lib().hvpr_spatial_gate_f32(_ptr(y_nhwc, torch.float32, "scale features"), N, H, W, C,
                                      _ptr(w18, torch.float32, "gate conv weight"), float(conv_bias), float(bn_scale),
                                      float(bn_shift), gate.data_ptr(), _stream()), "hvpr_spatial_gate_f32")
    return gate


def head_decode(head_nhwc, n_anchor, n_class, n_dir_bins, x_shifts, y_shifts, anchor_table, dir_offset, dir_limit_offset,
                period, want_cls=True, want_scores=True, out=None):
    N, H, W, CH = head_nhwc.shape
    A = H * W * n_anchor
    dev = head_nhwc.device
    if out is not None:
        cls, box, scores, labels = out
        if box.shape != (N, A, 7) or not all(t is None or t.is_contiguous() for t in out):
            raise ValueError("head_decode: `out` tensors do not match this call")
    else:
        cls = torch.empty((N, A, n_class), dtype=torch.float32, device=dev) if want_cls else None
        box = torch.empty((N, A, 7), dtype=torch.float32, device=dev)
        scores = torch.empty((N, A), dtype=torch.float32, device=dev) if want_scores else None
        labels = torch.empty((N, A), dtype=torch.int32, device=dev) if want_scores else None
    check(lib().hvpr_head_decode_f32(_ptr(head_nhwc, torch.float32, "head output"), N, H, W, CH, n_anchor, n_class,
                                     n_dir_bins, _ptr(x_shifts, torch.float32), _ptr(y_shifts, torch.float32),
                                     _ptr(anchor_table, torch.float32), float(dir_offset), float(dir_limit_offset),
                                     float(period), _ptr(cls), box.data_ptr(), _ptr(scores), _ptr(labels), _stream()),
          "hvpr_head_decode_f32")
    return cls, box, scores, labels


MAX_NMS_SEGMENTS = 16


class PostWorkspace:

    def __init__(self, batch, n_scores, pre_max, device, segments=None):
        self.batch, self.n_scores, self.pre_max = batch, n_scores, pre_max
        self.nms_segments = max(1, min(batch if segments is None else int(segments), MAX_NMS_SEGMENTS))
        self.topk = torch.zeros(lib().hvpr_score_topk_workspace_bytes(batch, n_scores), dtype=torch.uint8, device=device)
        self.nms = torch.empty(lib().hvpr_nms_bev_batched_workspace_bytes(self.nms_segments, pre_max), dtype=torch.uint8, device=device)


def score_topk(scores, score_thresh, pre_max, ws, want_scores=True):
    B, A = scores.shape
    if B != ws.batch:
        raise ValueError(f"score_topk: {B} frames on a workspace made for {ws.batch}")
    dev = scores.device
    order = torch.empty((B, pre_max), dtype=torch.int32, device=dev)
    ss = torch.empty((B, pre_max), dtype=torch.float32, device=dev) if want_scores else None
    counts = torch.empty((B,), dtype=torch.int32, device=dev)
    use = score_thresh is not None
    check(lib().hvpr_score_topk_f32(_ptr(scores, torch.float32, "scores"), B, A, float(score_thresh) if use else 0.0,
                                    1 if use else 0, int(pre_max), order.data_ptr(), _ptr(ss), counts.data_ptr(),
                                    ws.topk.data_ptr(), ws.topk.numel(), _stream()), "hvpr_score_topk_f32")
    return order, ss, counts


def nms_bev(boxes, order, n_device, n_max, thresh, max_keep, ws_nms, map_through_order=True):
    dev = boxes.device
    keep = torch.zeros((max(max_keep, 1),), dtype=torch.int32, device=dev)
    kc = torch.empty((1,), dtype=torch.int32, device=dev)
    check(lib().hvpr_nms_bev_f32(_ptr(boxes, torch.float32, "boxes"), boxes.shape[1], _ptr(order, torch.int32),
                                 _ptr(n_device, torch.int32), int(n_max), float(thresh), int(max_keep),
                                 1 if map_through_order else 0, keep.data_ptr(), kc.data_ptr(), ws_nms.data_ptr(),
                                 ws_nms.numel(), _stream()), "hvpr_nms_bev_f32")
    return keep, kc


def gather_predictions(boxes, scores, labels, keep):
    K = keep.shape[0]
    dev = boxes.device
    ob = torch.empty((K, 7), dtype=torch.float32, device=dev)
    os_ = torch.empty((K,), dtype=torch.float32, device=dev)
    ol = torch.empty((K,), dtype=torch.int64, device=dev)
    osel = torch.empty((K,), dtype=torch.int64, device=dev)
    check(lib().hvpr_gather_predictions_f32(_ptr(boxes, torch.float32, "boxes"), boxes.shape[1], _ptr(scores, torch.float32, "scores"),
                                            _ptr(labels, torch.int32, "labels"), _ptr(keep, torch.int32, "keep"), K, ob.data_ptr(),
                                            os_.data_ptr(), ol.data_ptr(), osel.data_ptr(), _stream()), "hvpr_gather_predictions_f32")
    return ob, os_, ol, osel


def nms_segment_chunks(n_tables, segments_per_table=1):
    cap, spt = max(int(MAX_NMS_SEGMENTS), 1), int(segments_per_table)
    if spt <= cap:
        step = cap // spt
        for t0 in range(0, n_tables, step):
            t1 = min(n_tables, t0 + step)
            yield t0 * spt, t1 * spt, t0, t1, spt
    else:
        for t in range(n_tables):
            for k0 in range(0, spt, cap):
                k1 = min(spt, k0 + cap)
                yield t * spt + k0, t * spt + k1, t, t + 1, k1 - k0


def nms_call_segments(n_tables, segments_per_table=1):
    return max((s1 - s0 for s0, s1, _, _, _ in nms_segment_chunks(n_tables, segments_per_table)), default=1)


def nms_bev_batched(boxes, order, n_device, n_max, thresh, max_keep, ws_nms, map_through_order=True, segments_per_table=1):
    if boxes.dim() != 3:
        raise ValueError("nms_bev_batched: boxes must be (tables, rows, >= 7)")
    S = boxes.shape[0] * int(segments_per_table)
    if order is not None and tuple(order.shape) != (S, n_max):
        raise ValueError(f"nms_bev_batched: order must be ({S}, {n_max}), got {tuple(order.shape)}")
    if n_device is not None and tuple(n_device.shape) != (S,):
        raise ValueError(f"nms_bev_batched: n_device must be ({S},), got {tuple(n_device.shape)}")
    dev = boxes.device
    keep = torch.zeros((S, max(max_keep, 1)), dtype=torch.int32, device=dev)
    kc = torch.empty((S,), dtype=torch.int32, device=dev)
    check(lib().hvpr_nms_bev_batched_f32(_ptr(boxes, torch.float32, "boxes"), boxes.shape[2], boxes.shape[1] * boxes.shape[2],
                                         int(segments_per_table), _ptr(order, torch.int32), _ptr(n_device, torch.int32), S, int(n_max),
                                         float(thresh), int(max_keep), 1 if map_through_order else 0, keep.data_ptr(), kc.data_ptr(),
                                         ws_nms.data_ptr(), ws_nms.numel(), _stream()), "hvpr_nms_bev_batched_f32")
    return keep, kc


def gather_predictions_batched(boxes, scores, labels, keep, segments_per_table=1):
    S, K = keep.shape
    if boxes.dim() != 3 or boxes.shape[0] * int(segments_per_table) != S or tuple(scores.shape) != (S, boxes.shape[1]) \
            or labels.shape != scores.shape:
        raise ValueError("gather_predictions_batched: shapes do not match")
    dev = boxes.device
    ob = torch.empty((S, K, 7), dtype=torch.float32, device=dev)
    os_ = torch.empty((S, K), dtype=torch.float32, device=dev)
    ol = torch.empty((S, K), dtype=torch.int64, device=dev)
    osel = torch.empty((S, K), dtype=torch.int64, device=dev)
    check(lib().hvpr_gather_predictions_batched_f32(_ptr(boxes, torch.float32, "boxes"), boxes.shape[2], boxes.shape[1] * boxes.shape[2],
                                                    int(segments_per_table), _ptr(scores, torch.float32, "scores"),
                                                    _ptr(labels, torch.int32, "labels"), scores.shape[1], _ptr(keep, torch.int32, "keep"),
                                                    S, K, ob.data_ptr(), os_.data_ptr(), ol.data_ptr(), osel.data_ptr(), _stream()),
          "hvpr_gather_predictions_batched_f32")
    return ob, os_, ol, osel


def gather_predictions_multiclass(boxes, scores, keep, keep_count, num_class):
    nc = int(num_class)
    S, K = keep.shape
    if boxes.dim() != 3 or nc < 1 or boxes.shape[0] * nc != S or tuple(scores.shape) != (S, boxes.shape[1]) \
            or tuple(keep_count.shape) != (S,):
        raise ValueError("gather_predictions_multiclass: shapes do not match")
    B, dev = boxes.shape[0], boxes.device
    ob = torch.empty((B, nc * K, 7), dtype=torch.float32, device=dev)
    os_ = torch.empty((B, nc * K), dtype=torch.float32, device=dev)
    ol = torch.empty((B, nc * K), dtype=torch.int64, device=dev)
    osel = torch.empty((B, nc * K), dtype=torch.int64, device=dev)
    oc = torch.empty((B,), dtype=torch.int32, device=dev)
    check(lib().hvpr_gather_predictions_multiclass_f32(_ptr(boxes, torch.float32, "boxes"), boxes.shape[2], boxes.shape[1] * boxes.shape[2],
                                                       _ptr(scores, torch.float32, "scores"), scores.shape[1],
                                                       _ptr(keep, torch.int32, "keep"), _ptr(keep_count, torch.int32, "keep_count"),
                                                       B, nc, K, ob.data_ptr(), os_.data_ptr(), ol.data_ptr(), osel.data_ptr(),
                                                       oc.data_ptr(), _stream()), "hvpr_gather_predictions_multiclass_f32")
    return ob, os_, ol, osel, oc


def boxes_pairwise(a, b, mode):
    a = a[:, :7].contiguous()
    b = b[:, :7].contiguous()
    out = torch.zeros((a.shape[0], b.shape[0]), dtype=torch.float32, device=a.device)
    check(lib().hvpr_boxes_pairwise_f32(_ptr(a, torch.float32, "boxes_a"), a.shape[0], _ptr(b, torch.float32, "boxes_b"),
                                        b.shape[0], int(mode), out.data_ptr(), _stream()), "hvpr_boxes_pairwise_f32")
    return out


def boxes_pairwise_ragged(a, b, a_off, b_off, pair_off, n_pairs):
    out = torch.empty((int(n_pairs),), dtype=torch.float32, device=pair_off.device)
    check(lib().hvpr_boxes_pairwise_ragged_f32(_ptr(a, torch.float32, "boxes_a"), _ptr(b, torch.float32, "boxes_b"),
                                               _ptr(a_off, torch.int64, "a_off"), _ptr(b_off, torch.int64, "b_off"),
                                               _ptr(pair_off, torch.int64, "pair_off"), pair_off.numel() - 1, int(n_pairs),
                                               out.data_ptr(), _stream()), "hvpr_boxes_pairwise_ragged_f32")
    return out


def kitti_overlaps(gt_rows, dt_rows, inter, gt_off, dt_off, pair_off, n_pairs, metric):
    out = torch.empty((int(n_pairs),), dtype=torch.float64, device=pair_off.device)
    check(lib().hvpr_kitti_overlaps_f64(_ptr(gt_rows, torch.float64, "gt_rows"), _ptr(dt_rows, torch.float64, "dt_rows"),
                                        _ptr(inter, torch.float32, "inter"), _ptr(gt_off, torch.int64, "gt_off"),
                                        _ptr(dt_off, torch.int64, "dt_off"), _ptr(pair_off, torch.int64, "pair_off"),
                                        pair_off.numel() - 1, int(n_pairs), int(metric), out.data_ptr(), _stream()),
          "hvpr_kitti_overlaps_f64")
    return out


def kitti_match(gt_rows, gt_cls, gt_dontcare, dt_rows, dt_cls, gt_off, dt_off, pair_off, overlaps, metric, classes, min_overlaps,
                thresholds=None, thresh_count=None, compute_aos=False, out=None):
    import ctypes
    dev = pair_off.device
    F, NG = pair_off.numel() - 1, gt_rows.shape[0]
    C, K = len(classes), len(min_overlaps)
    combos = C * 3 * K
    c_classes = (ctypes.c_int32 * C)(*[int(c) for c in classes])
    c_mo = (ctypes.c_double * (K * C))(*[float(v) for row in min_overlaps for v in row])
    if thresholds is None:
        a, b = out if out is not None else (torch.empty((combos, NG), dtype=torch.float64, device=dev),
                                            torch.empty((C, 3), dtype=torch.int32, device=dev))
        args = (None, None, 1, 0, _ptr(a, torch.float64, "tp_score"), _ptr(b, torch.int32, "n_valid"), None, None, None, 0)
    else:
        T = thresholds.shape[1]
        a, b = out if out is not None else (torch.empty((combos, T, 3), dtype=torch.int32, device=dev),
                                            torch.empty((combos, T), dtype=torch.float64, device=dev))
        ws = torch.empty((lib().hvpr_kitti_match_workspace_bytes(F, C, K, T),), dtype=torch.uint8, device=dev)
        args = (_ptr(thresholds, torch.float64, "thresholds"), _ptr(thresh_count, torch.int32, "thresh_count"), T, int(bool(compute_aos)),
                None, None, _ptr(a, torch.int32, "counts"), _ptr(b, torch.float64, "sim"), ws.data_ptr(), ws.numel())
    check(lib().hvpr_kitti_match_f64(_ptr(gt_rows, torch.float64, "gt_rows"), _ptr(gt_cls, torch.int32, "gt_cls"),
                                     _ptr(gt_dontcare, torch.uint8, "gt_dontcare"), _ptr(dt_rows, torch.float64, "dt_rows"),
                                     _ptr(dt_cls, torch.int32, "dt_cls"), _ptr(gt_off, torch.int64, "gt_off"),
                                     _ptr(dt_off, torch.int64, "dt_off"), _ptr(pair_off, torch.int64, "pair_off"), F, NG,
                                     _ptr(overlaps, torch.float64, "overlaps"), int(metric), 0 if thresholds is None else 1,
                                     c_classes, C, c_mo, K, *args, _stream()), "hvpr_kitti_match_f64")
    return a, b


def recall_record(pred_boxes, pred_count, gt_boxes, thresholds, counts=None, best_iou=None):
    import ctypes
    B, P = int(pred_boxes.shape[0]), int(pred_boxes.shape[1])
    if pred_boxes.dim() != 3 or pred_boxes.shape[2] != 7 or gt_boxes.dim() != 3 or gt_boxes.shape[0] != B or pred_count.numel() != B:
        raise ValueError("recall_record: pred_boxes (B, P, 7), pred_count (B,) and gt_boxes (B, G, C) must agree")
    G, C, T = int(gt_boxes.shape[1]), int(gt_boxes.shape[2]), len(thresholds)
    if counts is None:
        counts = torch.empty((B, 1 + T), dtype=torch.int32, device=pred_boxes.device)
    if tuple(counts.shape) != (B, 1 + T) or (best_iou is not None and tuple(best_iou.shape) != (B, G)):
        raise ValueError("recall_record: counts must be (B, 1 + T) and best_iou (B, G)")
    thr = (ctypes.c_float * max(T, 1))(*[float(t) for t in thresholds])
    check(lib().hvpr_recall_record_f32(_ptr(pred_boxes, torch.float32, "pred_boxes"), _ptr(pred_count, torch.int32, "pred_count"), B, P,
                                       _ptr(gt_boxes, torch.float32, "gt_boxes"), G, C, thr, T, _ptr(counts, torch.int32, "counts"),
                                       _ptr(best_iou, torch.float32, "best_iou"), _stream()), "hvpr_recall_record_f32")
    return counts


def prediction_annos(pred_boxes, pred_scores, pred_labels, pred_count, calib, class_of_label, row_base, frame_base, dt_rows, dt_cls,
                     dt_label, dt_box7, boxes_lidar, dt_off, overflow):
    import ctypes
    B, P = int(pred_boxes.shape[0]), int(pred_boxes.shape[1])
    if tuple(pred_boxes.shape) != (B, P, 7) or tuple(pred_scores.shape) != (B, P) or tuple(pred_labels.shape) != (B, P) \
            or pred_count.numel() != B or tuple(calib.shape) != (B, 26):
        raise ValueError("prediction_annos: shapes do not match")
    cap = int(dt_rows.shape[0])
    if tuple(dt_rows.shape) != (cap, 16) or dt_cls.numel() != cap or dt_label.numel() != cap or tuple(dt_box7.shape) != (cap, 7) \
            or tuple(boxes_lidar.shape) != (cap, 7):
        raise ValueError("prediction_annos: the tables must hold the same number of rows")
    n = len(class_of_label)
    cmap = (ctypes.c_int32 * max(n, 1))(*[int(c) for c in class_of_label])
    check(lib().hvpr_prediction_annos_f32(_ptr(pred_boxes, torch.float32, "pred_boxes"), _ptr(pred_scores, torch.float32, "pred_scores"),
                                          _ptr(pred_labels, torch.int64, "pred_labels"), _ptr(pred_count, torch.int32, "pred_count"),
                                          B, P, _ptr(calib, torch.float32, "calib"), cmap, n, _ptr(row_base, torch.int64, "row_base"),
                                          cap, int(frame_base), dt_off.numel() - 1, _ptr(dt_rows, torch.float64, "dt_rows"),
                                          _ptr(dt_cls, torch.int32, "dt_cls"), _ptr(dt_label, torch.int32, "dt_label"),
                                          _ptr(dt_box7, torch.float32, "dt_box7"), _ptr(boxes_lidar, torch.float32, "boxes_lidar"),
                                          _ptr(dt_off, torch.int64, "dt_off"), _ptr(overflow, torch.int32, "overflow"), _stream()),
          "hvpr_prediction_annos_f32")


def augment_block_points():
    return int(lib().hvpr_augment_block_points())


def augment_collide(plan_host, plan_dev, words):
    C = int(plan_host.numpy()[4])
    valid = torch.zeros((max(C, 1),), dtype=torch.int32, device=plan_dev.device)
    check(lib().hvpr_augment_collide_f32(plan_host.data_ptr(), _ptr(plan_dev, torch.int32, "plan"), int(words), valid.data_ptr(),
                                         _stream()), "hvpr_augment_collide_f32")
    return valid[:C]


def augment_boxes(plan_host, plan_dev, words, valid, point_cloud_range, remove_outside, g_cap, out=None, count=None):
    import numpy as np
    B = int(plan_host.numpy()[1])
    rng6 = np.ascontiguousarray(point_cloud_range, np.float32)
    if out is None:
        out = torch.empty((B, g_cap, 8), dtype=torch.float32, device=plan_dev.device)
    if count is None:
        count = torch.empty((B,), dtype=torch.int32, device=plan_dev.device)
    check(lib().hvpr_augment_boxes_f32(plan_host.data_ptr(), _ptr(plan_dev, torch.int32, "plan"), int(words),
                                       _ptr(valid, torch.int32, "valid"), rng6.ctypes.data, int(bool(remove_outside)), int(g_cap),
                                       _ptr(out, torch.float32, "gt_boxes"), _ptr(count, torch.int32, "count"), _stream()),
          "hvpr_augment_boxes_f32")
    return out, count


def augment_points(plan_host, plan_dev, words, valid, points, bank_points, bank_boxes, extra_width, out=None, out_off=None):
    import numpy as np
    h = plan_host.numpy()
    B, NG, G, C = int(h[1]), int(h[2]), int(h[3]), int(h[4])
    n, F = points.shape
    ex = np.ascontiguousarray(extra_width, np.float32)
    pt_off = h[8 + (B + 1) + (B * NG + 1):][: B + 1]
    max_frame = int(np.diff(pt_off).max()) if B > 0 else 0
    if out is None:
        c5 = 8 + (B + 1) + (B * NG + 1) + (B + 1) + G + 4 * C
        out = torch.empty((n + int(h[c5: c5 + C].sum()), F), dtype=torch.float32, device=points.device)
    if out_off is None:
        out_off = torch.empty((B + 1,), dtype=torch.int32, device=points.device)
    ws = _workspace(None, lib().hvpr_augment_points_workspace_bytes(B, max_frame, C, n), points.device)
    check(lib().hvpr_augment_points_f32(plan_host.data_ptr(), _ptr(plan_dev, torch.int32, "plan"), int(words),
                                        _ptr(valid, torch.int32, "valid"), _ptr(points, torch.float32, "points"), n, F,
                                        _ptr(bank_points, torch.float32, "bank points"), bank_points.shape[0],
                                        _ptr(bank_boxes, torch.float32, "bank boxes"), bank_boxes.shape[0], bank_points.shape[1],
                                        ex.ctypes.data, _ptr(out, torch.float32, "out_points"), out.shape[0],
                                        _ptr(out_off, torch.int32, "out_off"), ws.data_ptr(), ws.numel(), _stream()),
          "hvpr_augment_points_f32")
    return out, out_off


def augment_batch(plan_host, plan_dev, words, points, bank, extra_width, point_cloud_range, remove_outside, g_cap):
    B = int(plan_host.numpy()[1])
    arena, obj_box = bank.on_device()
    counts = torch.empty((2 * B + 1,), dtype=torch.int32, device=points.device)
    valid = augment_collide(plan_host, plan_dev, words)
    gt, _ = augment_boxes(plan_host, plan_dev, words, valid, point_cloud_range, remove_outside, g_cap, count=counts[B + 1:])
    pts, off = augment_points(plan_host, plan_dev, words, valid, points, arena, obj_box, extra_width, out_off=counts[: B + 1])
    return {"points": pts, "point_frame_offsets": off, "gt_boxes": gt, "valid": valid, "counts": counts}


def gt_database_block_points():
    return int(lib().hvpr_gt_database_block_points())


def _gt_database_workspace(pt_off_host, n_obj, device, workspace):
    import numpy as np
    off = pt_off_host.numpy()
    max_frame = int(np.diff(off).max()) if off.shape[0] > 1 else 0
    return _workspace(workspace, lib().hvpr_gt_database_workspace_bytes(off.shape[0] - 1, max_frame, int(n_obj)), device)


def gt_database_count(points, pt_off_host, pt_off, boxes, box_off_host, box_off, obj_count=None, workspace=None):
    n, F = points.shape
    n_obj, B = int(boxes.shape[0]), pt_off_host.numel() - 1
    if obj_count is None:
        obj_count = torch.empty((max(n_obj, 1),), dtype=torch.int32, device=points.device)[:n_obj]
    workspace = _gt_database_workspace(pt_off_host, n_obj, points.device, workspace)
    check(lib().hvpr_gt_database_count_f32(_ptr(points, torch.float32, "points"), n, F, pt_off_host.data_ptr(),
                                           _ptr(pt_off, torch.int32, "pt_off"), B, _ptr(boxes, torch.float32, "boxes"),
                                           box_off_host.data_ptr(), _ptr(box_off, torch.int32, "box_off"), n_obj,
                                           _ptr(obj_count, torch.int32, "obj_count"), workspace.data_ptr(), workspace.numel(), _stream()),
          "hvpr_gt_database_count_f32")
    return obj_count, workspace


def gt_database_extract(points, pt_off_host, pt_off, boxes, box_off_host, box_off, centres, obj_count_host, obj_count, arena,
                        workspace, obj_off=None):
    n, F = points.shape
    n_obj, B = int(boxes.shape[0]), pt_off_host.numel() - 1
    if arena.shape[1] != F:
        raise ValueError("gt_database_extract: the arena must have the points' feature width")
    if obj_off is None:
        obj_off = torch.empty((n_obj + 1,), dtype=torch.int32, device=points.device)
    check(lib().hvpr_gt_database_extract_f32(_ptr(points, torch.float32, "points"), n, F, pt_off_host.data_ptr(),
                                             _ptr(pt_off, torch.int32, "pt_off"), B, _ptr(boxes, torch.float32, "boxes"),
                                             box_off_host.data_ptr(), _ptr(box_off, torch.int32, "box_off"),
                                             _ptr(centres, torch.float64, "centres"), n_obj, obj_count_host.data_ptr(),
                                             _ptr(obj_count, torch.int32, "obj_count"), _ptr(obj_off, torch.int32, "obj_off"),
                                             _ptr(arena, torch.float32, "arena"), arena.shape[0], workspace.data_ptr(),
                                             workspace.numel(), _stream()), "hvpr_gt_database_extract_f32")
    return obj_off


def kitti_infos_block_points():
    return int(lib().hvpr_kitti_infos_block_points())


def kitti_infos_count(points, pt_off_host, pt_off, boxes, box_off_host, box_off, calib_host, calib, obj_count=None, fov_count=None,
                      want_fov=False, workspace=None):
    import numpy as np
    n, F = points.shape
    n_obj, B = int(boxes.shape[0]), pt_off_host.numel() - 1
    if calib_host.dtype != torch.float32 or calib_host.numel() != 26 * B or not calib_host.is_contiguous() or calib_host.is_cuda:
        raise ValueError("kitti_infos_count: calib_host must be a contiguous (B, 26) float32 host tensor")
    if calib.numel() != 26 * B:
        raise ValueError("kitti_infos_count: calib must be (B, 26)")
    if obj_count is None:
        obj_count = torch.empty((max(n_obj, 1),), dtype=torch.int32, device=points.device)[:n_obj]
    if fov_count is None and want_fov:
        fov_count = torch.empty((B,), dtype=torch.int32, device=points.device)
    off = pt_off_host.numpy()
    max_frame = int(np.diff(off).max()) if off.shape[0] > 1 else 0
    workspace = _workspace(workspace, lib().hvpr_kitti_infos_workspace_bytes(B, max_frame, n_obj), points.device)
    check(lib().hvpr_kitti_infos_count_f32(_ptr(points, torch.float32, "points"), n, F, pt_off_host.data_ptr(),
                                           _ptr(pt_off, torch.int32, "pt_off"), B, _ptr(boxes, torch.float32, "boxes"),
                                           box_off_host.data_ptr(), _ptr(box_off, torch.int32, "box_off"), n_obj,
                                           calib_host.data_ptr(), _ptr(calib, torch.float32, "calib"),
                                           _ptr(obj_count, torch.int32, "obj_count"), _ptr(fov_count, torch.int32, "fov_count"),
                                           workspace.data_ptr(), workspace.numel(), _stream()), "hvpr_kitti_infos_count_f32")
    return obj_count, fov_count, workspace


def ragged_select_tile_rows():
    return int(lib().hvpr_ragged_select_tile_rows())


def _workspace(workspace, need, device):
    if workspace is None or workspace.numel() < need:
        workspace = torch.empty((max(int(need), 256),), dtype=torch.uint8, device=device)
    return workspace


def _ragged_head(points, off, mask, calib, range_xy):
    import numpy as np
    rows, F = points.shape
    B = off.numel() - 1
    r = None if range_xy is None else np.ascontiguousarray(range_xy, np.float32).reshape(4)
    head = (_ptr(points, torch.float32, "points"), rows, F, _ptr(off, torch.int32, "off"), B, int(mask),
            _ptr(calib, torch.float32, "calib"), None if r is None else r.ctypes.data)
    return rows, F, B, head, r


def _offsets(t, B, device):
    return torch.empty((B + 1,), dtype=torch.int32, device=device) if t is None else t


def _out_and_flag(out, flag, rows, width, device):
    if out is None:
        out = torch.empty((rows, width), dtype=torch.float32, device=device)
    if flag is None:
        flag = torch.zeros((1,), dtype=torch.int32, device=device)
    return out, flag


def ragged_select_count(points, off, mask, calib=None, range_xy=None, new_off=None, workspace=None):
    rows, F, B, head, _r = _ragged_head(points, off, mask, calib, range_xy)
    new_off = _offsets(new_off, B, points.device)
    workspace = _workspace(workspace, lib().hvpr_ragged_select_workspace_bytes(rows, B), points.device)
    check(lib().hvpr_ragged_select_count_f32(*head, _ptr(new_off, torch.int32, "new_off"), workspace.data_ptr(),
                                             workspace.numel(), _stream()), "hvpr_ragged_select_count_f32")
    return new_off, workspace


def ragged_select_write(points, off, mask, new_off, workspace, calib=None, range_xy=None, inv_perm=None, batch_column=False,
                        out=None, flag=None):
    rows, F, B, head, _r = _ragged_head(points, off, mask, calib, range_xy)
    out, flag = _out_and_flag(out, flag, rows, F + (1 if batch_column else 0), points.device)
    check(lib().hvpr_ragged_select_write_f32(*head, _ptr(new_off, torch.int32, "new_off"), _ptr(inv_perm, torch.int32, "inv_perm"),
                                             0 if inv_perm is None else inv_perm.numel(), int(bool(batch_column)),
                                             _ptr(out, torch.float32, "out"), out.shape[0], _ptr(flag, torch.int32, "flag"),
                                             workspace.data_ptr(), workspace.numel(), _stream()), "hvpr_ragged_select_write_f32")
    return out, flag


def ragged_sample_count(points, off, mask, calib=None, range_xy=None, near=40.0, new_off=None, near_off=None, workspace=None):
    rows, F, B, head, _r = _ragged_head(points, off, mask, calib, range_xy)
    new_off, near_off = _offsets(new_off, B, points.device), _offsets(near_off, B, points.device)
    workspace = _workspace(workspace, lib().hvpr_ragged_sample_workspace_bytes(rows, B), points.device)
    check(lib().hvpr_ragged_sample_count_f32(*head, float(near), _ptr(new_off, torch.int32, "new_off"),
                                             _ptr(near_off, torch.int32, "near_off"), workspace.data_ptr(), workspace.numel(),
                                             _stream()), "hvpr_ragged_sample_count_f32")
    return new_off, near_off, workspace


def ragged_sample_write(points, off, mask, new_off, near_off, mode, dest, num_points, workspace, calib=None, range_xy=None,
                        near=40.0, batch_column=False, out=None, flag=None):
    rows, F, B, head, _r = _ragged_head(points, off, mask, calib, range_xy)
    out, flag = _out_and_flag(out, flag, B * int(num_points), F + (1 if batch_column else 0), points.device)
    if mode.numel() != B or dest.dim() != 2 or dest.shape[1] != 2:
        raise ValueError("hvpr_amd: mode must be (B,) and dest (n, 2)")
    check(lib().hvpr_ragged_sample_write_f32(*head, float(near), _ptr(new_off, torch.int32, "new_off"),
                                             _ptr(near_off, torch.int32, "near_off"), _ptr(mode, torch.int32, "mode"),
                                             _ptr(dest, torch.int32, "dest"), dest.shape[0], int(num_points),
                                             int(bool(batch_column)), _ptr(out, torch.float32, "out"), out.shape[0],
                                             _ptr(flag, torch.int32, "flag"), workspace.data_ptr(), workspace.numel(), _stream()),
          "hvpr_ragged_sample_write_f32")
    return out, flag


def bev_grid(point_cloud_range, pixel):
    import numpy as np
    r = np.ascontiguousarray(point_cloud_range, np.float32).reshape(6)
    g = np.round((r[3:5] - r[:2]) / np.float32(pixel)).astype(np.int64)
    return int(g[1]), int(g[0])


def render_bev(points, frame_offsets, point_cloud_range, pixel, palette, tables=(), xyz_col=0, thickness=2, heading_sign=-1,
               image=None, counts=None, want_counts=False, workspace=None):
    import numpy as np
    tables = list(tables)
    if len(tables) > 2:
        raise ValueError("render_bev: two box tables at the most")
    if points.dim() != 2 or frame_offsets.dim() != 1 or frame_offsets.numel() < 2:
        raise ValueError("render_bev: points must be (n, stride) and frame_offsets (B + 1,)")
    n, stride = points.shape
    B = frame_offsets.numel() - 1
    rng = np.ascontiguousarray(point_cloud_range, np.float32).reshape(6)
    H, W = bev_grid(rng, pixel)
    need = lib().hvpr_render_bev_workspace_bytes(B, H, W)
    if need == 0:
        raise ValueError(f"render_bev: a picture of {B} x {H} x {W} pixels is not supported")
    dev = points.device
    if palette.dim() != 2 or palette.shape[1] != 3:
        raise ValueError("render_bev: palette must be (n_ink, 3)")
    if image is None:
        image = torch.empty((B, H, W, 3), dtype=torch.uint8, device=dev)
    elif tuple(image.shape) != (B, H, W, 3):
        raise ValueError(f"render_bev: image must be {(B, H, W, 3)}")
    if counts is None and want_counts:
        counts = torch.empty((B, H, W), dtype=torch.int32, device=dev)
    elif counts is not None and tuple(counts.shape) != (B, H, W):
        raise ValueError(f"render_bev: counts must be {(B, H, W)}")
    args = []
    for t in tables + [None] * (2 - len(tables)):
        if t is None:
            args += [None, 0, 7, None, None, 0.0, None, 0]
            continue
        boxes = t["boxes"]
        if boxes.dim() != 3 or boxes.shape[0] != B or boxes.shape[2] < 7:
            raise ValueError("render_bev: boxes must be (B, P, >= 7)")
        P = boxes.shape[1]
        for key, shape in (("count", (B,)), ("scores", (B, P)), ("labels", (B, P))):
            if t.get(key) is not None and tuple(t[key].shape) != shape:
                raise ValueError(f"render_bev: {key} must be {shape}")
        args += [_ptr(boxes, torch.float32, "boxes") if P else None, P, boxes.shape[2], _ptr(t.get("count"), torch.int32, "count"),
                 _ptr(t.get("scores"), torch.float32, "scores"), float(t.get("thresh", 0.0)),
                 _ptr(t.get("labels"), torch.int64, "labels"), int(t.get("ink", 1))]
    workspace = _workspace(workspace, need, dev)
    check(lib().hvpr_render_bev_u8(_ptr(points, torch.float32, "points") if n else None, n, stride, int(xyz_col),
                                   _ptr(frame_offsets, torch.int32, "frame_offsets"), B, rng.ctypes.data, float(pixel), *args,
                                   _ptr(palette, torch.uint8, "palette"), palette.shape[0], int(thickness), int(heading_sign),
                                   _ptr(image, torch.uint8, "image"), _ptr(counts, torch.int32, "counts"), workspace.data_ptr(),
                                   workspace.numel(), _stream()), "hvpr_render_bev_u8")
    return image, counts, workspace
```

include/hvpr_amd.h:

```cpp
#ifndef HVPR_AMD_H
#define HVPR_AMD_H

#include <stddef.h>
#include <stdint.h>

#ifdef __cplusplus
extern "C" {
#endif

typedef void *hvpr_stream_t;

enum hvpr_status {
    HVPR_OK = 0,
    HVPR_ERR_INVALID_ARG = -1,
    HVPR_ERR_UNSUPPORTED = -2,
    HVPR_ERR_WORKSPACE = -3,
    HVPR_ERR_LAUNCH = -4,
    HVPR_ERR_TIMEOUT = -5
};

int hvpr_abi_version(void);
const char *hvpr_status_string(int status);

typedef int (*hvpr_allreduce_fn)(double *buf, int n, hvpr_stream_t stream, void *ctx);
void hvpr_set_batchnorm_allreduce(hvpr_allreduce_fn fn, void *ctx);

size_t hvpr_voxelize_workspace_bytes(int max_batch, int max_points, int nx, int ny, int nz);
int hvpr_voxelize_workspace_reset(void *workspace, size_t workspace_bytes, int max_batch, int max_points, int nx, int ny,
                                  int nz, hvpr_stream_t stream);
int hvpr_voxelize_workspace_status(const void *workspace, size_t workspace_bytes, int max_batch, int max_points, int nx, int ny,
                                   int nz, hvpr_stream_t stream);
int hvpr_voxelize_f32(const float *points, int n_points, int point_stride, int xyz_col, int n_feat,
                      const int32_t *frame_offsets, int batch, float lo_x, float lo_y, float lo_z, float vs_x,
                      float vs_y, float vs_z, int nx, int ny, int nz, int max_points, int max_voxels, int cap_mode,
                      float *voxels, int32_t *coords, int32_t *num_points, int32_t *voxel_offsets, int capacity,
                      void *workspace, size_t workspace_bytes, int ws_max_batch, int ws_max_points,
                      hvpr_stream_t stream);

int hvpr_pillar_vfe_fwd_f32(const float *voxels, const int32_t *num_points, const int32_t *coords, int M, int P,
                            const int32_t *m_device, float vs_x, float vs_y, float vs_z, float off_x, float off_y,
                            float off_z, const float *w0, const float *b0, const float *w1, const float *b1,
                            const float *ws0, const float *bs0, const float *ws1, const float *bs1,
                            float *pillar_features, float *pillar_scale_features, float *pillar_mask,
                            hvpr_stream_t stream);

size_t hvpr_pillar_vfe_train_workspace_bytes(void);
int hvpr_pillar_vfe_train_fwd_f32(const float *voxels, const int32_t *num_points, const int32_t *coords, int M, int P, const float *w0,
                                  const float *gamma0, const float *beta0, const float *w1, const float *gamma1, const float *beta1,
                                  float eps, float vs_x, float vs_y, float vs_z, float off_x, float off_y, float off_z,
                                  float *pillar_features, float *mean0, float *var0, float *mean1, float *var1, void *workspace,
                                  size_t workspace_bytes, hvpr_stream_t stream);
int hvpr_pillar_vfe_bwd_f32(const float *voxels, const int32_t *num_points, const int32_t *coords, int M, int P, const float *w0,
                            const float *gamma0, const float *beta0, const float *w1, const float *gamma1, const float *beta1, float eps,
                            float vs_x, float vs_y, float vs_z, float off_x, float off_y, float off_z, const float *d_pillar_features,
                            float *dw0, float *dgamma0, float *dbeta0, float *dw1, float *dgamma1, float *dbeta1, void *workspace,
                            size_t workspace_bytes, hvpr_stream_t stream);

size_t hvpr_memory_bank_packed_floats(int n_items);
int hvpr_memory_bank_pack_f32(const float *bank, int n_items, float *packed, hvpr_stream_t stream);
int hvpr_memory_readout_fwd_f32(const float *f, int M, const int32_t *m_device, const float *bank, const float *bank_packed,
                                int n_items, int k, float *out, int32_t *topk_idx, hvpr_stream_t stream);

size_t hvpr_scatter_workspace_bytes(int batch, int nx, int ny);
int hvpr_scatter_bev_fwd_f32(const float *pillar_features, int c_pillar, const float *memory_features, int c_mem,
                             const float *scale_features, int c_scale, const int32_t *coords, int M,
                             const int32_t *m_device, int batch, int nx, int ny, float *spatial,
                             float *spatial_scale, void *workspace, size_t workspace_bytes, hvpr_stream_t stream);

int hvpr_memory_scatter_fwd_f32(const float *pillar_features, const float *scale_features, const int32_t *coords, int M,
                                const int32_t *m_device, const float *bank, const float *bank_packed, int n_items, int k, int batch,
                                int nx, int ny,
                                float *memory_features, float *spatial, float *spatial_scale, void *workspace,
                                size_t workspace_bytes, hvpr_stream_t stream);

int hvpr_encode_fwd_f32(const float *points, int n_points, int point_stride, int xyz_col, int n_feat,
                        const int32_t *frame_offsets, int batch, float lo_x, float lo_y, float lo_z, float vs_x, float vs_y,
                        float vs_z, int nx, int ny, int nz, int max_points, int max_voxels, int cap_mode, float off_x,
                        float off_y, float off_z, const float *w0, const float *b0, const float *w1, const float *b1,
                        const float *ws0, const float *bs0, const float *ws1, const float *bs1, const float *bank,
                        const float *bank_packed, int n_items, int k, float *voxels, int32_t *coords, int32_t *num_points, int32_t *voxel_offsets,
                        int capacity, float *pillar_features, float *pillar_scale_features, float *pillar_mask,
                        float *memory_features, float *spatial, float *spatial_scale, uint8_t *canvas_state, void *workspace,
                        size_t workspace_bytes, int ws_max_batch, int ws_max_points, int index_mode, hvpr_stream_t stream);

int hvpr_conv2d_nhwc_f32(const float *in, int N, int H, int W, int Cin, const float *w_packed, const float *bias,
                         int taps, int stride, int cout, int cout_pad, int up, int relu, const float *gate,
                         const float *resid, int resid_cstride, float *out, int out_cstride, int out_coff,
                         int tile_cfg, hvpr_stream_t stream);
size_t hvpr_conv2d_tab_bytes(int N, int H, int W, int taps, int stride, int cout_pad, int tile_cfg);
int hvpr_conv2d_tab_build(int N, int H, int W, int taps, int stride, int cout_pad, int tile_cfg, void *table, hvpr_stream_t stream);
int hvpr_conv2d_nhwc_tab_f32(const float *in, int N, int H, int W, int Cin, const float *w_packed, const float *bias,
                             int taps, int stride, int cout, int cout_pad, int up, int relu, const float *gate,
                             const float *resid, int resid_cstride, float *out, int out_cstride, int out_coff,
                             int tile_cfg, const void *table, hvpr_stream_t stream);

int hvpr_spatial_gate_f32(const float *y, int N, int H, int W, int C, const float *w18, float conv_bias, float bn_scale,
                          float bn_shift, float *gate, hvpr_stream_t stream);

int hvpr_head_decode_f32(const float *head, int N, int H, int W, int head_channels, int n_anchor, int n_class,
                         int n_dir_bins, const float *x_shifts, const float *y_shifts, const float *anchor_table,
                         float dir_offset, float dir_limit_offset, float period, float *batch_cls_preds,
                         float *batch_box_preds, float *scores, int32_t *labels, hvpr_stream_t stream);

size_t hvpr_score_topk_workspace_bytes(int batch, int n_scores);
int hvpr_score_topk_f32(const float *scores, int batch, int n_scores, float score_thresh, int use_thresh, int pre_max,
                        int32_t *order, float *sorted_scores, int32_t *counts, void *workspace, size_t workspace_bytes,
                        hvpr_stream_t stream);

size_t hvpr_nms_workspace_bytes(int n_max);
int hvpr_nms_bev_f32(const float *boxes, int box_stride, const int32_t *order, const int32_t *n_device, int n_max,
                     float thresh, int max_keep, int map_through_order, int32_t *keep, int32_t *keep_count,
                     void *workspace, size_t workspace_bytes, hvpr_stream_t stream);
int hvpr_gather_predictions_f32(const float *boxes, int box_stride, const float *scores, const int32_t *labels,
                                const int32_t *keep, int max_keep, float *out_boxes, float *out_scores, int64_t *out_labels,
                                int64_t *out_selected, hvpr_stream_t stream);
int hvpr_boxes_pairwise_f32(const float *boxes_a, int n, const float *boxes_b, int m, int mode, float *out,
                            hvpr_stream_t stream);

size_t hvpr_nms_bev_batched_workspace_bytes(int n_segments, int n_max);
int hvpr_nms_bev_batched_f32(const float *boxes, int box_stride, long long table_stride, int segments_per_table,
                             const int32_t *order, const int32_t *n_device, int n_segments, int n_max, float thresh,
                             int max_keep, int map_through_order, int32_t *keep, int32_t *keep_count, void *workspace,
                             size_t workspace_bytes, hvpr_stream_t stream);
int hvpr_gather_predictions_batched_f32(const float *boxes, int box_stride, long long table_stride, int segments_per_table,
                                        const float *scores, const int32_t *labels, long long score_stride,
                                        const int32_t *keep, int n_segments, int max_keep, float *out_boxes,
                                        float *out_scores, int64_t *out_labels, int64_t *out_selected, hvpr_stream_t stream);
int hvpr_gather_predictions_multiclass_f32(const float *boxes, int box_stride, long long table_stride, const float *scores,
                                           long long score_stride, const int32_t *keep, const int32_t *keep_count, int n_frames,
                                           int n_class, int max_keep, float *out_boxes, float *out_scores, int64_t *out_labels,
                                           int64_t *out_selected, int32_t *out_count, hvpr_stream_t stream);

int hvpr_boxes_pairwise_ragged_f32(const float *boxes_a, const float *boxes_b, const int64_t *a_off, const int64_t *b_off,
                                   const int64_t *pair_off, int n_frames, long long n_pairs, float *out, hvpr_stream_t stream);
int hvpr_kitti_overlaps_f64(const double *gt_rows, const double *dt_rows, const float *inter, const int64_t *gt_off,
                            const int64_t *dt_off, const int64_t *pair_off, int n_frames, long long n_pairs, int metric,
                            double *out, hvpr_stream_t stream);
size_t hvpr_kitti_match_workspace_bytes(int n_frames, int n_classes, int n_sets, int n_thresh);
int hvpr_kitti_match_f64(const double *gt_rows, const int32_t *gt_cls, const uint8_t *gt_dontcare, const double *dt_rows,
                         const int32_t *dt_cls, const int64_t *gt_off, const int64_t *dt_off, const int64_t *pair_off,
                         int n_frames, long long n_gt_total, const double *overlaps, int metric, int pass,
                         const int32_t *classes, int n_classes, const double *min_overlaps, int n_sets,
                         const double *thresholds, const int32_t *thresh_count, int n_thresh, int compute_aos,
                         double *tp_score, int32_t *n_valid, int32_t *counts, double *sim, void *workspace,
                         size_t workspace_bytes, hvpr_stream_t stream);

int hvpr_recall_record_f32(const float *pred_boxes, const int32_t *pred_count, int B, int P, const float *gt_boxes, int G, int C,
                           const float *thresholds, int T, int32_t *counts, float *best_iou, hvpr_stream_t stream);
int hvpr_prediction_annos_f32(const float *pred_boxes, const float *pred_scores, const int64_t *pred_labels,
                              const int32_t *pred_count, int B, int P, const float *calib, const int32_t *class_of_label,
                              int n_labels, int64_t *row_base, long long cap, int frame_base, int max_frames, double *dt_rows,
                              int32_t *dt_cls, int32_t *dt_label, float *dt_box7, float *boxes_lidar, int64_t *dt_off,
                              int32_t *overflow, hvpr_stream_t stream);

int hvpr_furthest_point_sample_f32(const float *xyz, int B, int N, int npoint, int32_t *idx, hvpr_stream_t stream);
int hvpr_ball_query_f32(const float *xyz, const float *new_xyz, int B, int N, int M, float radius, int nsample, int32_t *idx,
                        hvpr_stream_t stream);
int hvpr_three_nn_f32(const float *unknown, const float *known, int B, int n, int m, float *dist, int32_t *idx,
                      hvpr_stream_t stream);

int hvpr_group_points_f32(const float *features, const int32_t *idx, int B, int C, int N, int npoint, int nsample, float *out,
                          hvpr_stream_t stream);
int hvpr_three_interpolate_f32(const float *features, const int32_t *idx, const float *weight, int B, int C, int m, int n,
                               float *out, hvpr_stream_t stream);
int hvpr_group_rows_f32(const float *xyz, const float *features, const float *new_xyz, const int32_t *idx, int B, int N, int C,
                        int npoint, int nsample, int cpad, float *out, hvpr_stream_t stream);
int hvpr_max_samples_f32(const float *y, long long G, int nsample, int C, float *out, uint8_t *argmax, hvpr_stream_t stream);
int hvpr_max_samples_grad_f32(const float *grad_out, const uint8_t *argmax, long long G, int nsample, int C, float *grad_y,
                              hvpr_stream_t stream);
int hvpr_fp_rows_f32(const float *known, const int32_t *idx, const float *weight, const float *skip, int B, int m, int n, int C1,
                     int C2, int cpad, float *out, hvpr_stream_t stream);
size_t hvpr_spatial_gate_train_workspace_bytes(int N, int H, int W);
int hvpr_spatial_gate_train_fwd_f32(const float *y, int N, int H, int W, int C, const float *w18, const float *conv_bias,
                                    const float *gamma, const float *beta, float eps, float *pooled, int32_t *argmax, float *a,
                                    float *stats, float *gate, void *workspace, size_t workspace_bytes, hvpr_stream_t stream);
int hvpr_spatial_gate_train_bwd_f32(const float *dgate, const float *gate, const float *a, const float *stats, const float *pooled,
                                    const int32_t *argmax, const float *w18, const float *gamma, int N, int H, int W, int C,
                                    float *dy, float *dw18, float *dbias, float *dgamma, float *dbeta, void *workspace,
                                    size_t workspace_bytes, hvpr_stream_t stream);
int hvpr_point_pillar_topk_f32(const float *pillars, int M, const float *points, const float *points_packed, int N, int k,
                               int32_t *idx, hvpr_stream_t stream);

int hvpr_segment_sum_rows_f32(const float *src, long long src_stride, int src_off, int C, const int32_t *edge_row,
                              const float *edge_w, const int32_t *rowptr, long long n_dst, float *dst, long long dst_stride,
                              hvpr_stream_t stream);

int hvpr_attend_rows_fwd_f32(const float *q, int M, const float *rows, long long N, const int32_t *idx, int k, int C, float *out,
                             float *w, hvpr_stream_t stream);

size_t hvpr_memory_train_workspace_bytes(int n_items);
int hvpr_memory_train_fwd_f32(const float *x, long long R, const float *bank, int n_items, float shrink_thres, float *y, float *row_stats,
                              void *workspace, size_t workspace_bytes, hvpr_stream_t stream);
int hvpr_memory_train_bwd_f32(const float *x, const float *dy, long long R, const float *bank, int n_items, float shrink_thres,
                              const float *row_stats, float *dx, float *dbank, float *row_scratch, void *workspace,
                              size_t workspace_bytes, hvpr_stream_t stream);

size_t hvpr_conv2d_wino_wgrad_workspace_bytes(int N, int H, int W, int Cin, int Cout);
int hvpr_conv2d_wino_wgrad_nhwc_f32(const float *x, int N, int H, int W, int Cin, const float *dz, int Cout, float *dw,
                                    void *workspace, size_t workspace_bytes, hvpr_stream_t stream);
size_t hvpr_conv2d_wgrad_workspace_bytes(int N, int OH, int OW, int Cin, int Cout, int taps, int stride);
int hvpr_conv2d_wgrad_nhwc_f32(const float *x, int N, int H, int W, int Cin, const float *dz, int Cout, int taps, int stride, float *dw,
                               void *workspace, size_t workspace_bytes, hvpr_stream_t stream);
int hvpr_conv2d_s2_dgrad_nhwc_f32(const float *dz, int N, int H, int W, int Cin, const float *w_packed, const float *bias, int cout,
                                  int cout_pad, int OH, int OW, float *dx, int out_cstride, int out_coff, hvpr_stream_t stream);

size_t hvpr_bn_workspace_bytes(long long P, int C);
int hvpr_bn_stats_nhwc_f32(const float *z, long long P, int C, float eps, float *mean, float *var, float *invstd, void *workspace,
                           size_t workspace_bytes, hvpr_stream_t stream);
int hvpr_bn_finalize_partials_f32(const float *partials, int rows, int C, long long count, float eps, float *mean, float *var,
                                  float *invstd, hvpr_stream_t stream);
int hvpr_bn_train_affine_f32(const float *mean, const float *var, const float *invstd, int C, const float *gamma, const float *beta,
                             float momentum, float momentum_unbiased, float *running_mean, float *running_var,
                             long long *num_batches_tracked, float *scale, float *shift, hvpr_stream_t stream);
int hvpr_bn_relu_fwd_nhwc_f32(const float *z, long long P, int C, const float *scale, const float *shift, int relu, const float *gate,
                              const float *resid, float *y, int y_cstride, int y_coff, hvpr_stream_t stream);
int hvpr_bn_relu_bwd_sums_nhwc_f32(const float *dy, int dy_cstride, int dy_coff, const float *z, long long P, int C, const float *scale,
                                   const float *shift, const float *mean, const float *invstd, int relu, const float *gate, float *dgamma,
                                   float *dbeta, void *workspace, size_t workspace_bytes, hvpr_stream_t stream);
int hvpr_bn_relu_bwd_apply_nhwc_f32(const float *dy, int dy_cstride, int dy_coff, const float *z, long long P, int C, const float *scale,
                                    const float *shift, const float *mean, const float *invstd, int relu, const float *gate, float *dgate,
                                    float *dz, const float *dgamma_total, const float *dbeta_total, double inv_count, hvpr_stream_t stream);

size_t hvpr_assign_targets_workspace_bytes(int batch, int n_gt);
int hvpr_assign_targets_f32(const float *anchors, int n_anchors, const float *gt_boxes, int batch, int n_gt, int class_index,
                            int n_classes, float matched_thr, float unmatched_thr, int per_loc, int loc_stride, int loc_offset,
                            long long anchors_total, int32_t *labels, float *reg_targets, float *reg_weights, int32_t *pos_count,
                            void *workspace, size_t workspace_bytes, hvpr_stream_t stream);

size_t hvpr_rpn_losses_workspace_bytes(int batch, long long n_anchors);
int hvpr_rpn_losses_f32(const float *cls_preds, const float *box_preds, const float *dir_preds, const int32_t *labels,
                        const float *reg_targets, const float *anchor_rot, const int32_t *pos_count, int batch, long long n_anchors,
                        int num_class, int num_dir_bins, float alpha, float gamma, float beta, const float *code_weights,
                        float cls_weight, float loc_weight, float dir_weight, float dir_offset, float *losses, float *grad_cls,
                        float *grad_box, float *grad_dir, void *workspace, size_t workspace_bytes, hvpr_stream_t stream);
size_t hvpr_mse_loss_workspace_bytes(void);
int hvpr_mse_loss_f32(const float *x, const float *target, long long rows, int cols, float weight, float *loss, float *grad_x,
                      void *workspace, size_t workspace_bytes, hvpr_stream_t stream);

int hvpr_fused_adam_truewd_f32(float *params, const float *grads, float *exp_avg, float *exp_avg_sq, long long n, float lr,
                               float beta1, float beta2, float eps, float weight_decay, int step,
                               const float *grad_scale_device, hvpr_stream_t stream);
int hvpr_fused_adam_l2_f32(float *params, const float *grads, float *exp_avg, float *exp_avg_sq, long long n, float lr, float beta1,
                           float beta2, float eps, float weight_decay, int step, const float *grad_scale_device,
                           hvpr_stream_t stream);
int hvpr_fused_sgd_f32(float *params, const float *grads, float *momentum_buf, long long n, float lr, float momentum,
                       float weight_decay, const float *grad_scale_device, hvpr_stream_t stream);


size_t hvpr_conv2d_wino_packed_floats(int cin, int cout);
int hvpr_conv2d_wino_pack_f32(const float *weight, const float *scale, int cout, int cin, int adjoint, float *packed,
                              hvpr_stream_t stream);
int hvpr_conv2d_wino_nhwc_f32(const float *in, int N, int H, int W, int Cin, const float *w_packed, const float *bias, int cout,
                              int relu, const float *gate, const float *resid, int resid_cstride, float *out, int out_cstride,
                              int out_coff, int px_groups, float *bn_partials, hvpr_stream_t stream);
int hvpr_conv2d_wino_stats_rows(int N, int H, int W);
int hvpr_conv2d_wino_items(int N, int H, int W, int cout, int px_groups);
size_t hvpr_conv2d_wino_tab_bytes(int N, int H, int W, int cout, int px_groups);
int hvpr_conv2d_wino_tab_build(int N, int H, int W, int cout, int px_groups, void *table, hvpr_stream_t stream);
int hvpr_conv2d_wino_nhwc_tab_f32(const float *in, int N, int H, int W, int Cin, const float *w_packed, const float *bias, int cout,
                                  int relu, const float *gate, const float *resid, int resid_cstride, float *out, int out_cstride,
                                  int out_coff, int px_groups, float *bn_partials, const void *table, hvpr_stream_t stream);

int hvpr_split_bf16_f32(const float *src, long long n_floats, int n_planes, void *dst, hvpr_stream_t stream);
int hvpr_unsplit_bf16_f32(const void *src, long long n_floats, int n_planes, float *dst, hvpr_stream_t stream);
int hvpr_conv2d_nhwc_bf16x3(const void *in_split, int N, int H, int W, int Cin, const void *w_split, const float *bias,
                            int stride, int cout, int cout_pad, int relu, const float *gate, const void *resid_split,
                            int resid_cstride, void *out, int out_split, int out_cstride, int out_coff, int tile_cfg,
                            int n_planes, hvpr_stream_t stream);
int hvpr_deconv_nhwc_bf16x3(const void *in_split, int N, int H, int W, int Cin, const void *w_split, const float *bias, int cout,
                            int cout_pad, int up, int relu, float *out, int out_cstride, int out_coff, int n_planes,
                            hvpr_stream_t stream);

int hvpr_point_flags_f32(const float *points, int n, int stride, int mode, const float *range_xy, float near_thresh,
                         const float *fov_lidar_to_rect, const float *fov_rect_to_img, int img_h, int img_w, uint8_t *flags,
                         hvpr_stream_t stream);
size_t hvpr_compact_workspace_bytes(int n);
int hvpr_compact_rows_f32(const float *src, int n, int row_floats, const uint8_t *flags, float *dst, int capacity,
                          int32_t *count, void *workspace, size_t workspace_bytes, hvpr_stream_t stream);
int hvpr_gather_rows_f32(const float *src, int n_src, int row_floats, const int32_t *idx, int m, float *dst,
                         hvpr_stream_t stream);
int hvpr_frame_offsets_f32(const float *points, int n_points, int point_stride, int batch, int32_t *frame_offsets,
                           hvpr_stream_t stream);

int hvpr_augment_block_points(void);
int hvpr_augment_collide_f32(const int32_t *plan_host, const int32_t *plan_dev, int plan_words, int32_t *valid,
                             hvpr_stream_t stream);
int hvpr_augment_boxes_f32(const int32_t *plan_host, const int32_t *plan_dev, int plan_words, const int32_t *valid,
                           const float *range6, int remove_outside, int g_cap, float *gt_out, int32_t *box_count,
                           hvpr_stream_t stream);
size_t hvpr_augment_points_workspace_bytes(int n_frames, int max_frame_points, int n_candidates, long long n_points);
int hvpr_augment_points_f32(const int32_t *plan_host, const int32_t *plan_dev, int plan_words, const int32_t *valid,
                            const float *points, long long n_points, int point_floats, const float *bank_points,
                            long long bank_rows, const float *bank_boxes, int n_objects, int bank_floats,
                            const float *extra_width3, float *out_points, long long out_capacity, int32_t *out_off,
                            void *workspace, size_t workspace_bytes, hvpr_stream_t stream);

int hvpr_gt_database_block_points(void);
size_t hvpr_gt_database_workspace_bytes(int n_frames, int max_frame_points, int n_obj);
int hvpr_gt_database_count_f32(const float *points, long long n_points, int point_floats, const int32_t *pt_off_host,
                               const int32_t *pt_off, int n_frames, const float *boxes, const int32_t *box_off_host,
                               const int32_t *box_off, int n_obj, int32_t *obj_count, void *workspace, size_t workspace_bytes,
                               hvpr_stream_t stream);
int hvpr_gt_database_extract_f32(const float *points, long long n_points, int point_floats, const int32_t *pt_off_host,
                                 const int32_t *pt_off, int n_frames, const float *boxes, const int32_t *box_off_host,
                                 const int32_t *box_off, const double *centres, int n_obj, const int32_t *obj_count_host,
                                 const int32_t *obj_count, int32_t *obj_off, float *arena, long long arena_capacity,
                                 void *workspace, size_t workspace_bytes, hvpr_stream_t stream);

int hvpr_ragged_select_tile_rows(void);
size_t hvpr_ragged_select_workspace_bytes(long long rows, int n_frames);
int hvpr_ragged_select_count_f32(const float *points, long long rows, int point_floats, const int32_t *off, int n_frames,
                                 int mask, const float *calib, const float *range_xy, int32_t *new_off, void *workspace,
                                 size_t workspace_bytes, hvpr_stream_t stream);
int hvpr_ragged_select_write_f32(const float *points, long long rows, int point_floats, const int32_t *off, int n_frames,
                                 int mask, const float *calib, const float *range_xy, const int32_t *new_off,
                                 const int32_t *inv_perm, long long n_perm, int batch_column, float *out,
                                 long long out_capacity, int32_t *flag, void *workspace, size_t workspace_bytes,
                                 hvpr_stream_t stream);

size_t hvpr_ragged_sample_workspace_bytes(long long rows, int n_frames);
int hvpr_ragged_sample_count_f32(const float *points, long long rows, int point_floats, const int32_t *off, int n_frames,
                                 int mask, const float *calib, const float *range_xy, float near, int32_t *new_off,
                                 int32_t *near_off, void *workspace, size_t workspace_bytes, hvpr_stream_t stream);
int hvpr_ragged_sample_write_f32(const float *points, long long rows, int point_floats, const int32_t *off, int n_frames,
                                 int mask, const float *calib, const float *range_xy, float near, const int32_t *new_off,
                                 const int32_t *near_off, const int32_t *mode, const int32_t *dest, long long n_dest,
                                 int num_points, int batch_column, float *out, long long out_capacity, int32_t *flag,
                                 void *workspace, size_t workspace_bytes, hvpr_stream_t stream);

int hvpr_kitti_infos_block_points(void);
size_t hvpr_kitti_infos_workspace_bytes(int n_frames, int max_frame_points, int n_obj);
int hvpr_kitti_infos_count_f32(const float *points, long long n_points, int point_floats, const int32_t *pt_off_host,
                               const int32_t *pt_off, int n_frames, const float *boxes, const int32_t *box_off_host,
                               const int32_t *box_off, int n_obj, const float *calib_host, const float *calib,
                               int32_t *obj_count, int32_t *fov_count, void *workspace, size_t workspace_bytes,
                               hvpr_stream_t stream);

size_t hvpr_render_bev_workspace_bytes(int batch, int height, int width);
int hvpr_render_bev_u8(const float *points, long long n_points, int point_stride, int xyz_col, const int32_t *frame_offsets,
                       int batch, const float *range, float pixel, const float *boxes0, int rows0, int box_stride0,
                       const int32_t *count0, const float *scores0, float thresh0, const long long *labels0, int ink0,
                       const float *boxes1, int rows1, int box_stride1, const int32_t *count1, const float *scores1,
                       float thresh1, const long long *labels1, int ink1, const uint8_t *palette, int n_ink, int thickness,
                       int heading_sign, uint8_t *image, int32_t *counts, void *workspace, size_t workspace_bytes,
                       hvpr_stream_t stream);

#ifdef __cplusplus
}
#endif
#endif
```

Before: 463.2 frames/s.

## Walk 1x1 convolutions as flat pixel runs and add narrow-N head tile

Adds a RUN mode to the implicit-GEMM conv kernel so that 1x1 convolutions treat the NHWC input as one flat run of pixels rather than 2D spatial tiles. This removes border and halo handling and the partial edge tiles. A new tile configuration uses a 4x1 wave grid with BN equal to cout_pad (32/64/96), and the anchor head uses it so its small output channel count is not padded to 64. Upsampled outputs recover (n, oy, ox) through magic-number division, and walk tables gain a run encoding. The risks are extra template instantiations and a different wave split that could lower MFMA efficiency.

```diff
diff --git a/hvpr_amd/_lib.py b/hvpr_amd/_lib.py
--- a/hvpr_amd/_lib.py
+++ b/hvpr_amd/_lib.py
@@ -111,6 +111,9 @@
     "hvpr_conv2d_tab_bytes": (_Z, [_I, _I, _I, _I, _I, _I, _I]),
     "hvpr_conv2d_tab_build": (_I, [_I, _I, _I, _I, _I, _I, _I, _P, _P]),
     "hvpr_conv2d_nhwc_tab_f32": (_I, [_P, _I, _I, _I, _I, _P, _P, _I, _I, _I, _I, _I, _I, _P, _P, _I, _P, _I, _I, _I, _P, _P]),
+    "hvpr_conv2d_run_tab_bytes": (_Z, [_I, _I, _I, _I, _I]),
+    "hvpr_conv2d_run_tab_build": (_I, [_I, _I, _I, _I, _I, _P, _P]),
+    "hvpr_conv2d_run_nhwc_f32": (_I, [_P, _I, _I, _I, _I, _P, _P, _I, _I, _I, _I, _P, _P, _I, _P, _I, _I, _I, _P, _P]),
     "hvpr_conv2d_s2_dgrad_nhwc_f32": (_I, [_P, _I, _I, _I, _I, _P, _P, _I, _I, _I, _I, _P, _I, _I, _P]),
     "hvpr_bn_train_affine_f32": (_I, [_P, _P, _P, _I, _P, _P, _F, _F, _P, _P, _P, _P, _P, _P]),
     "hvpr_bn_finalize_partials_f32": (_I, [_P, _I, _I, _c.c_longlong, _F, _P, _P, _P, _P]),
diff --git a/hvpr_amd/anchor_head.py b/hvpr_amd/anchor_head.py
--- a/hvpr_amd/anchor_head.py
+++ b/hvpr_amd/anchor_head.py
@@ -195,7 +195,8 @@
         w = torch.cat([c.weight.detach().float() for c in convs], dim=0)
         b = torch.cat([c.bias.detach().float() for c in convs], dim=0)
         x, y, table = self._decode_tables(device)
-        return {"pc": kernels.pack_conv(w, None, b, relu=False, tile_cfg=1), "xs": x, "ys": y, "table": table}
+        tile_cfg = 3 if w.shape[0] <= kernels.HEAD_TILE_MAX_COLUMNS else 1
+        return {"pc": kernels.pack_conv(w, None, b, relu=False, tile_cfg=tile_cfg), "xs": x, "ys": y, "table": table}
 
     def _forward_train(self, data_dict):
         from . import conv_train as ct
diff --git a/hvpr_amd/csrc/conv_igemm.hip b/hvpr_amd/csrc/conv_igemm.hip
--- a/hvpr_amd/csrc/conv_igemm.hip
+++ b/hvpr_amd/csrc/conv_igemm.hip
@@ -1,6 +1,7 @@
 #include <type_traits>
 
 #include "common.h"
+#include "conv_walk.h"
 
 namespace {
 
@@ -36,6 +37,8 @@
     int cout_real;
     int tiles_x, tiles_y, n_ct;
     const unsigned long long *tab;
+    int hw, total_px;
+    ConvDiv by_hw, by_ow;
 };
 
 enum { OPT_TAB = 1, OPT_PEEL = 2 };
@@ -52,13 +55,17 @@
 __device__ long long g_conv_dbg[8 * 4 * 64 * 4];
 #endif
 
-template <int TH, int TW, int BN, int S, int TAPS, bool UP2 = false, int OPT = 0>
+template <int TH, int TW, int BN, int S, int TAPS, bool UP2 = false, int OPT = 0, bool RUN = false, int WGN = 2>
 __global__ void __launch_bounds__(256) k_conv(ConvArgs a) {
     static_assert(!UP2 || (TAPS == 9 && S == 1 && TH == 16 && TW == 16), "UP2: 16 x 16 output tiles of a 3x3 stride-2 layer's data gradient");
     static_assert(!UP2 || OPT == 0, "the item switches belong to the forward instantiations");
     constexpr bool TAB = (OPT & OPT_TAB) != 0, PEEL = (OPT & OPT_PEEL) != 0;
+    static_assert(!RUN || (TAB && (TAPS == 1 || TAPS == 4) && S == 1), "the run walk: halo-free layers, items from a table");
+    static_assert((WGN == 2 || WGN == 1) && (WGN == 2 || !UP2), "wave grid 2 x 2 or 4 x 1");
     constexpr int BM = TH * TW;
-    constexpr int WM = BM / 2, WN = BN / 2;
+    constexpr int WGM = 4 / WGN;
+    static_assert(TH % WGM == 0 && BN % (32 * WGN) == 0, "a wave owns whole tile rows and whole 32-column blocks");
+    constexpr int WM = BM / WGM, WN = BN / WGN;
     constexpr int MB = WM / 32, NB = WN / 32;
     static_assert(MB >= 1 && NB >= 1, "wave tile must hold at least one 32x32 block");
     constexpr int HALO = TAPS == 9 ? 2 : 0;
@@ -77,7 +84,7 @@
 
     const int tid = threadIdx.x, lane = tid & 63, wid = tid >> 6;
     const unsigned wave_s = __builtin_amdgcn_readfirstlane((unsigned)(threadIdx.x >> 6));
-    const int wm = wid >> 1, wn = wid & 1;
+    const int wm = wid / WGN, wn = wid % WGN;
     const int half = lane >> 5, l31 = lane & 31;
 
     int p_py[NLD_P], p_px[NLD_P], p_part[NLD_P];
@@ -87,6 +94,7 @@
         const int v = tid + i * 256;
         const int part = v / PPAD, pix = v % PPAD;
         p_py[i] = pix / PW; p_px[i] = pix % PW; p_part[i] = part * 4;
+        if (RUN) { p_py[i] = pix; p_px[i] = 0; }
         p_live[i] = v < PATCH_V4 && pix < PH * PW;
     }
     unsigned woff0[NLD_W];
@@ -106,7 +114,7 @@
 #pragma unroll
     for (int mb = 0; mb < MB; ++mb) {
         const int q = mb * 32 + l31;
-        const int py = wm * (TH / 2) + q / TW, px = q % TW;
+        const int py = wm * (TH / WGM) + q / TW, px = q % TW;
         a_off[mb] = half * PPAD + (py * S) * PW + px * S;
         if (UP2) a_off[mb] = half * PPAD + (wm * 4 + (l31 >> 3)) * PW + (l31 & 7);
     }
@@ -116,7 +124,7 @@
     const unsigned lds_patch0 = lds_addr_of(&s_patch[0][0]) + wave_s * 1024u;
     const unsigned lds_w0 = lds_addr_of(&s_w[0][0]) + wave_s * 1024u;
 
-    const int n_pt = a.tiles_x * a.tiles_y * a.N;
+    const int n_pt = RUN ? a.tiles_x : a.tiles_x * a.tiles_y * a.N;
     const int total_walk = ((n_pt + 7) / 8) * 8 * a.n_ct;
 #ifdef HVPR_EXP_TIMING
     int dbg_tile = 0;
@@ -125,13 +133,22 @@
     unsigned long long e_next = 0ull;
     if (TAB && (int)blockIdx.x < total_walk) e_next = tab_load(a.tab, blockIdx.x);
     for (int it = blockIdx.x; it < total_walk; it += gridDim.x) {
-    int ct, tx, ty, n;
+    int ct, tx = 0, ty = 0, n;
+    int rem0 = 0, m0 = 0, live_px = BM;
     if constexpr (TAB) {
         const unsigned lo = (unsigned)e_next, hi = (unsigned)(e_next >> 32);
         if (it + (int)gridDim.x < total_walk) e_next = tab_load(a.tab, it + (int)gridDim.x);
         if (lo >> 31) continue;
-        tx = (int)(lo & 0xffffu); ty = (int)(lo >> 16 & 0x7fffu); ct = (int)(hi & 0xfffu); n = (int)(hi >> 12);
+        ct = (int)(hi & 0xfffu); n = (int)(hi >> 12);
         if (n >= a.N || ct >= a.n_ct) continue;
+        if constexpr (RUN) {
+            rem0 = (int)(lo & 0x7fffffffu);
+            if (rem0 >= a.hw) continue;
+            m0 = n * a.hw + rem0;
+            live_px = a.total_px - m0 < BM ? a.total_px - m0 : BM;
+        } else {
+            tx = (int)(lo & 0xffffu); ty = (int)(lo >> 16 & 0x7fffu);
+        }
     } else {
         const int xcd = it & 7, j = it >> 3;
         ct = j % a.n_ct;
@@ -149,12 +166,17 @@
     bool pok[NLD_P];
 #pragma unroll
     for (int i = 0; i < NLD_P; ++i) {
+        if constexpr (RUN) {
+            pok[i] = p_live[i] && p_py[i] < live_px;
+            poff[i] = pok[i] ? (unsigned)((p_py[i] * a.Cin + p_part[i]) * (int)sizeof(float)) : 0u;
+            continue;
+        }
         const int iy = iy0 + p_py[i], ix = ix0 + p_px[i];
         pok[i] = p_live[i] && iy >= 0 && iy < a.H && ix >= 0 && ix < a.W;
         poff[i] = pok[i] ? (unsigned)(((iy * a.W + ix) * a.Cin + p_part[i]) * (int)sizeof(float)) : 0u;
     }
     const unsigned w_co0 = (unsigned)(co0 * 4 * sizeof(float));
-    const char *in_n = (const char *)(a.in + (size_t)n * a.H * a.W * a.Cin);
+    const char *in_n = (const char *)(a.in + (RUN ? (size_t)m0 : (size_t)n * a.H * a.W) * a.Cin);
 
     auto stage_piece = [&](int chunk, int buf, int i) {
         if (i < NLD_P) {
@@ -171,7 +193,7 @@
         for (int i = 0; i < NLD_P + NLD_W; ++i) stage_piece(chunk, buf, i);
     };
     constexpr int DEAL = TAPS == 9 ? 6 : (TAPS == 4 ? 3 : 0);
-    const bool border = iy0 < 0 || ix0 < 0 || iy0 + PH > a.H || ix0 + PW > a.W;
+    const bool border = RUN ? live_px < BM : iy0 < 0 || ix0 < 0 || iy0 + PH > a.H || ix0 + PW > a.W;
     if (border) {
 #pragma unroll
         for (int b = 0; b < 2; ++b)
@@ -277,10 +299,22 @@
 #pragma unroll
     for (int mb = 0; mb < MB; ++mb) {
         const int q = mb * 32 + l31;
-        const int oy = UP2 ? oy0 + 2 * (wm * 4 + (l31 >> 3)) + (mb >> 1) : oy0 + wm * (TH / 2) + q / TW;
-        const int ox = UP2 ? ox0 + 2 * (l31 & 7) + (mb & 1) : ox0 + q % TW;
-        if (oy >= a.OH || ox >= a.OW) continue;
-        const size_t pix = ((size_t)n * a.OH + oy) * a.OW + ox;
+        int oy = UP2 ? oy0 + 2 * (wm * 4 + (l31 >> 3)) + (mb >> 1) : oy0 + wm * (TH / WGM) + q / TW;
+        int ox = UP2 ? ox0 + 2 * (l31 & 7) + (mb & 1) : ox0 + q % TW;
+        int on = n;
+        size_t pix;
+        if constexpr (RUN) {
+            const int j = wm * WM + q;
+            if (j >= live_px) continue;
+            pix = (size_t)m0 + j;
+            if (a.up > 1) {
+                const ConvRunPixel px = conv_run_pixel(n, rem0, j, a.hw, a.OW, a.by_hw, a.by_ow);
+                on = px.n; oy = px.oy; ox = px.ox;
+            }
+        } else {
+            if (oy >= a.OH || ox >= a.OW) continue;
+            pix = ((size_t)n * a.OH + oy) * a.OW + ox;
+        }
         const float gate = a.gate ? a.gate[pix] : 0.f;
         const float *rrow = a.gate ? a.resid + pix * a.resid_cstride : nullptr;
 #pragma unroll
@@ -299,7 +333,7 @@
                     const float4 r = *(const float4 *)(rrow + co);
                     y.x = fmaf(gate, y.x, r.x); y.y = fmaf(gate, y.y, r.y); y.z = fmaf(gate, y.z, r.z); y.w = fmaf(gate, y.w, r.w);
                 }
-                const size_t opix = a.up > 1 ? ((size_t)n * a.OH * a.up + (oy * a.up + sy)) * ((size_t)a.OW * a.up) + (ox * a.up + sx) : pix;
+                const size_t opix = a.up > 1 ? ((size_t)on * a.OH * a.up + (oy * a.up + sy)) * ((size_t)a.OW * a.up) + (ox * a.up + sx) : pix;
                 *(float4 *)(a.out + opix * a.out_cstride + a.out_coff + co) = y;
             }
         }
@@ -311,14 +345,17 @@
     }
 }
 
-__global__ void k_conv_tab(int N, int tiles_x, int tiles_y, int n_ct, int total_walk, unsigned long long *__restrict__ tab) {
+__global__ void k_conv_tab(int N, int tiles_x, int tiles_y, int n_ct, int total_walk, int run_px, int hw, unsigned long long *__restrict__ tab) {
     const int it = blockIdx.x * blockDim.x + threadIdx.x;
     if (it >= total_walk) return;
-    const int xcd = it & 7, j = it >> 3;
-    const int ct = j % n_ct;
-    int pt = (j / n_ct) * 8 + xcd;
+    int ct;
+    int pt = conv_walk_step(it, n_ct, ct);
+    if (run_px > 0) {
+        tab[it] = conv_run_entry(pt, tiles_x, run_px, hw, ct);
+        return;
+    }
     if (pt >= tiles_x * tiles_y * N) {
-        tab[it] = 1ull << 31;
+        tab[it] = CONV_TAB_HOLE;
         return;
     }
     const int tx = pt % tiles_x; pt /= tiles_x;
@@ -327,35 +364,59 @@
     tab[it] = (unsigned long long)((unsigned)tx | (unsigned)ty << 16) | (unsigned long long)((unsigned)ct | (unsigned)n << 12) << 32;
 }
 
-static int conv_tab_grid(int N, int H, int W, int taps, int stride, int cout_pad, int tile_cfg, int &tiles_x, int &tiles_y, int &n_ct) {
-    if (N < 1 || H < 1 || W < 1 || cout_pad < 1 || (taps != 9 && taps != 1) || (stride != 1 && stride != 2) || tile_cfg < 0 || tile_cfg > 2) return 0;
+struct ConvGrid {
+    int tiles_x, tiles_y, n_ct, run_px;
+};
+static int conv_tab_grid(int N, int H, int W, int taps, int stride, int cout_pad, int tile_cfg, bool run, ConvGrid &g) {
+    if (N < 1 || H < 1 || W < 1 || cout_pad < 1 || (taps != 9 && taps != 1) || (stride != 1 && stride != 2) || tile_cfg < 0 || tile_cfg > (run ? 3 : 2)) return 0;
+    if (run && (taps != 1 || stride != 1)) return 0;
+    if (tile_cfg == 3 && cout_pad > 96) return 0;
     const int OH = taps == 9 ? (H + 2 - 3) / stride + 1 : H, OW = taps == 9 ? (W + 2 - 3) / stride + 1 : W;
-    const int tw = tile_cfg == 1 ? 8 : 16, bn = tile_cfg == 0 ? 128 : 64;
-    if (OH < 1 || OW < 1 || cout_pad % bn != 0) return 0;
-    tiles_x = (OW + tw - 1) / tw; tiles_y = (OH + 7) / 8; n_ct = cout_pad / bn;
-    if (tiles_x > TAB_MAX_TX || tiles_y > TAB_MAX_TY || n_ct > TAB_MAX_CT || N > TAB_MAX_N) return 0;
-    const long long steps = ((long long)N * tiles_x * tiles_y + 7) / 8 * 8 * n_ct;
+    const int tw = tile_cfg == 1 ? 8 : 16, bn = tile_cfg == 0 ? 128 : (tile_cfg == 3 ? cout_pad : 64);
+    if (OH < 1 || OW < 1 || cout_pad % bn != 0 || bn % 32 != 0) return 0;
+    g.tiles_x = (OW + tw - 1) / tw; g.tiles_y = (OH + 7) / 8; g.n_ct = cout_pad / bn; g.run_px = 0;
+    if (g.tiles_x > TAB_MAX_TX || g.tiles_y > TAB_MAX_TY || g.n_ct > TAB_MAX_CT || N > TAB_MAX_N) return 0;
+    long long pixel_tiles = (long long)N * g.tiles_x * g.tiles_y;
+    if (run) {
+        const long long total_px = (long long)N * OH * OW;
+        if (total_px >= (1ll << 31) - 8 * tw) return 0;
+        g.run_px = 8 * tw;
+        pixel_tiles = (total_px + g.run_px - 1) / g.run_px;
+        g.tiles_x = (int)pixel_tiles; g.tiles_y = 1;
+    }
+    const long long steps = (pixel_tiles + 7) / 8 * 8 * g.n_ct;
     return steps < (1ll << 28) ? (int)steps : 0;
 }
 
-template <int TH, int TW, int BN, int S, int TAPS, bool UP2 = false, int OPT = 0>
+template <int TH, int TW, int BN, int S, int TAPS, bool UP2 = false, int OPT = 0, bool RUN = false, int WGN = 2>
 int launch(ConvArgs a, hipStream_t s) {
     a.tiles_x = (a.OW + TW - 1) / TW;
     a.tiles_y = (a.OH + TH - 1) / TH;
     a.n_ct = a.cout_pad / BN;
-    const long long tiles = (long long)a.N * a.tiles_x * a.tiles_y * a.n_ct;
+    long long tiles = (long long)a.N * a.tiles_x * a.tiles_y * a.n_ct;
+    a.hw = a.OH * a.OW;
+    a.total_px = 0;
+    a.by_hw = a.by_ow = ConvDiv{0ull, 0};
+    if (RUN) {
+        a.total_px = a.N * a.hw;
+        a.tiles_x = (a.total_px + TH * TW - 1) / (TH * TW);
+        a.tiles_y = 1;
+        a.by_hw = conv_div_make(a.hw);
+        a.by_ow = conv_div_make(a.OW);
+        tiles = (long long)a.tiles_x * a.n_ct;
+    }
     static int resident = 0;
     if (resident == 0) {
         int per_cu = 0, dev = 0, cus = 256;
         hipDeviceProp_t prop;
         if (hipGetDevice(&dev) == hipSuccess && hipGetDeviceProperties(&prop, dev) == hipSuccess) cus = prop.multiProcessorCount;
-        if (hipOccupancyMaxActiveBlocksPerMultiprocessor(&per_cu, k_conv<TH, TW, BN, S, TAPS, UP2, OPT>, 256, 0) != hipSuccess || per_cu < 1)
+        if (hipOccupancyMaxActiveBlocksPerMultiprocessor(&per_cu, k_conv<TH, TW, BN, S, TAPS, UP2, OPT, RUN, WGN>, 256, 0) != hipSuccess || per_cu < 1)
             per_cu = 1;
         resident = per_cu * cus;
     }
     long long blocks = tiles < resident ? (tiles + 7) / 8 * 8 : resident;
     if (blocks > resident && resident >= 8) blocks = resident / 8 * 8;
-    hipLaunchKernelGGL((k_conv<TH, TW, BN, S, TAPS, UP2, OPT>), dim3((unsigned)blocks), dim3(256), 0, s, a);
+    hipLaunchKernelGGL((k_conv<TH, TW, BN, S, TAPS, UP2, OPT, RUN, WGN>), dim3((unsigned)blocks), dim3(256), 0, s, a);
     return 0;
 }
 
@@ -385,26 +446,39 @@
     return HVPR_OK;
 }
 
-extern "C" size_t hvpr_conv2d_tab_bytes(int N, int H, int W, int taps, int stride, int cout_pad, int tile_cfg) {
-    int tiles_x, tiles_y, n_ct;
-    return (size_t)conv_tab_grid(N, H, W, taps, stride, cout_pad, tile_cfg, tiles_x, tiles_y, n_ct) * sizeof(unsigned long long);
-}
-
-extern "C" int hvpr_conv2d_tab_build(int N, int H, int W, int taps, int stride, int cout_pad, int tile_cfg, void *table, hvpr_stream_t stream) {
+static int conv_tab_build(int N, int H, int W, int taps, int stride, int cout_pad, int tile_cfg, bool run, void *table, hvpr_stream_t stream) {
     if (!table) return HVPR_ERR_INVALID_ARG;
-    int tiles_x, tiles_y, n_ct;
-    const int steps = conv_tab_grid(N, H, W, taps, stride, cout_pad, tile_cfg, tiles_x, tiles_y, n_ct);
+    ConvGrid g;
+    const int steps = conv_tab_grid(N, H, W, taps, stride, cout_pad, tile_cfg, run, g);
     if (steps == 0) return HVPR_ERR_UNSUPPORTED;
-    hipLaunchKernelGGL(k_conv_tab, dim3(hvpr_cdiv(steps, 256)), dim3(256), 0, (hipStream_t)stream, N, tiles_x, tiles_y, n_ct, steps,
-                       (unsigned long long *)table);
+    hipLaunchKernelGGL(k_conv_tab, dim3(hvpr_cdiv(steps, 256)), dim3(256), 0, (hipStream_t)stream, N, g.tiles_x, g.tiles_y, g.n_ct, steps,
+                       g.run_px, H * W, (unsigned long long *)table);
     HVPR_CHECK_LAUNCH();
     return HVPR_OK;
+}
+
+extern "C" size_t hvpr_conv2d_tab_bytes(int N, int H, int W, int taps, int stride, int cout_pad, int tile_cfg) {
+    ConvGrid g;
+    return (size_t)conv_tab_grid(N, H, W, taps, stride, cout_pad, tile_cfg, false, g) * sizeof(unsigned long long);
+}
+
+extern "C" int hvpr_conv2d_tab_build(int N, int H, int W, int taps, int stride, int cout_pad, int tile_cfg, void *table, hvpr_stream_t stream) {
+    return conv_tab_build(N, H, W, taps, stride, cout_pad, tile_cfg, false, table, stream);
+}
+
+extern "C" size_t hvpr_conv2d_run_tab_bytes(int N, int H, int W, int cout_pad, int tile_cfg) {
+    ConvGrid g;
+    return (size_t)conv_tab_grid(N, H, W, 1, 1, cout_pad, tile_cfg, true, g) * sizeof(unsigned long long);
+}
+
+extern "C" int hvpr_conv2d_run_tab_build(int N, int H, int W, int cout_pad, int tile_cfg, void *table, hvpr_stream_t stream) {
+    return conv_tab_build(N, H, W, 1, 1, cout_pad, tile_cfg, true, table, stream);
 }
 
 static int conv_nhwc(const float *in, int N, int H, int W, int Cin, const float *w_packed,
                      const float *bias, int taps, int stride, int cout, int cout_pad, int up,
                      int relu, const float *gate, const float *resid, int resid_cstride, float *out,
-                     int out_cstride, int out_coff, int tile_cfg, const void *table, hvpr_stream_t stream) {
+                     int out_cstride, int out_coff, int tile_cfg, const void *table, bool flat, hvpr_stream_t stream) {
     if (!in || !w_packed || !bias || !out || N < 1 || H < 1 || W < 1 || Cin < 8 || cout < 1) return HVPR_ERR_INVALID_ARG;
     if ((gate == nullptr) != (resid == nullptr)) return HVPR_ERR_INVALID_ARG;
     if (Cin % KC != 0 || (taps != 9 && taps != 1) || (stride != 1 && stride != 2) || up < 1) return HVPR_ERR_UNSUPPORTED;
@@ -424,24 +498,35 @@
     a.relu = relu; a.up = up;
     a.tab = (HVPR_ITEM_OPT & OPT_TAB) ? (const unsigned long long *)table : nullptr;
     if (cout_pad < a.cout_gemm) return HVPR_ERR_INVALID_ARG;
-    if (table && hvpr_conv2d_tab_bytes(N, H, W, taps, stride, cout_pad, tile_cfg) == 0) return HVPR_ERR_UNSUPPORTED;
+    ConvGrid grid;
+    if (table && conv_tab_grid(N, H, W, taps, stride, cout_pad, tile_cfg, flat, grid) == 0) return HVPR_ERR_UNSUPPORTED;
     hipStream_t s = (hipStream_t)stream;
-    const int bn = tile_cfg == 0 ? 128 : 64;
+    if (tile_cfg < 0 || tile_cfg > (flat ? 3 : 2)) return HVPR_ERR_INVALID_ARG;
+    const int bn = tile_cfg == 0 ? 128 : (tile_cfg == 3 ? cout_pad : 64);
     if (cout_pad % bn != 0) return HVPR_ERR_INVALID_ARG;
+    if (tile_cfg == 3 && (up != 1 || cout_pad % 32 != 0 || cout_pad > 96)) return HVPR_ERR_UNSUPPORTED;
     constexpr int OPT0 = HVPR_ITEM_OPT & ~OPT_TAB;
+    const bool run = flat && a.tab;
+#define HV_FLAT(TH, TW, BN, WGN)                                                            \
+    if (run && wide1x1) launch<TH, TW, BN, 1, 4, false, OPT0 | OPT_TAB, true, WGN>(a, s);   \
+    else if (run) launch<TH, TW, BN, 1, 1, false, OPT0 | OPT_TAB, true, WGN>(a, s);         \
+    else if (wide1x1) launch<TH, TW, BN, 1, 4, false, OPT0, false, WGN>(a, s);              \
+    else launch<TH, TW, BN, 1, 1, false, OPT0, false, WGN>(a, s);
 #define HV_CASE(TH, TW, BN, OPT)                                                    \
     if (taps == 9 && stride == 1) launch<TH, TW, BN, 1, 9, false, OPT>(a, s);       \
-    else if (taps == 9 && stride == 2) launch<TH, TW, BN, 2, 9, false, OPT>(a, s);  \
-    else if (wide1x1) launch<TH, TW, BN, 1, 4, false, OPT>(a, s);                   \
-    else launch<TH, TW, BN, 1, 1, false, OPT>(a, s);
+    else launch<TH, TW, BN, 2, 9, false, OPT>(a, s);
 #define HV_TILE(TH, TW, BN)                                                         \
-    if (a.tab) { HV_CASE(TH, TW, BN, OPT0 | OPT_TAB) } else { HV_CASE(TH, TW, BN, OPT0) }
+    if (taps == 1) { HV_FLAT(TH, TW, BN, 2) }                                       \
+    else if (a.tab) { HV_CASE(TH, TW, BN, OPT0 | OPT_TAB) } else { HV_CASE(TH, TW, BN, OPT0) }
     if (tile_cfg == 0) { HV_TILE(8, 16, 128) }
     else if (tile_cfg == 1) { HV_TILE(8, 8, 64) }
     else if (tile_cfg == 2) { HV_TILE(8, 16, 64) }
-    else return HVPR_ERR_INVALID_ARG;
+    else if (cout_pad == 32) { HV_FLAT(8, 16, 32, 1) }
+    else if (cout_pad == 64) { HV_FLAT(8, 16, 64, 1) }
+    else { HV_FLAT(8, 16, 96, 1) }
 #undef HV_TILE
 #undef HV_CASE
+#undef HV_FLAT
     HVPR_CHECK_LAUNCH();
     return HVPR_OK;
 }
@@ -451,7 +536,7 @@
                                     int relu, const float *gate, const float *resid, int resid_cstride, float *out,
                                     int out_cstride, int out_coff, int tile_cfg, hvpr_stream_t stream) {
     return conv_nhwc(in, N, H, W, Cin, w_packed, bias, taps, stride, cout, cout_pad, up, relu, gate, resid, resid_cstride, out, out_cstride,
-                     out_coff, tile_cfg, nullptr, stream);
+                     out_coff, tile_cfg, nullptr, false, stream);
 }
 
 extern "C" int hvpr_conv2d_nhwc_tab_f32(const float *in, int N, int H, int W, int Cin, const float *w_packed,
@@ -459,5 +544,12 @@
                                         int relu, const float *gate, const float *resid, int resid_cstride, float *out,
                                         int out_cstride, int out_coff, int tile_cfg, const void *table, hvpr_stream_t stream) {
     return conv_nhwc(in, N, H, W, Cin, w_packed, bias, taps, stride, cout, cout_pad, up, relu, gate, resid, resid_cstride, out, out_cstride,
-                     out_coff, tile_cfg, table, stream);
-}
+                     out_coff, tile_cfg, table, false, stream);
+}
+
+extern "C" int hvpr_conv2d_run_nhwc_f32(const float *in, int N, int H, int W, int Cin, const float *w_packed, const float *bias, int cout,
+                                        int cout_pad, int up, int relu, const float *gate, const float *resid, int resid_cstride,
+                                        float *out, int out_cstride, int out_coff, int tile_cfg, const void *table, hvpr_stream_t stream) {
+    return conv_nhwc(in, N, H, W, Cin, w_packed, bias, 1, 1, cout, cout_pad, up, relu, gate, resid, resid_cstride, out, out_cstride, out_coff,
+                     tile_cfg, table, true, stream);
+}
diff --git a/hvpr_amd/csrc/conv_walk.h b/hvpr_amd/csrc/conv_walk.h
--- /dev/null
+++ b/hvpr_amd/csrc/conv_walk.h
@@ -0,0 +1,55 @@
+#pragma once
+
+#ifndef HVPR_WALK_HD
+#if defined(__HIPCC__) || defined(__CUDACC__)
+#define HVPR_WALK_HD __host__ __device__ __forceinline__
+#else
+#define HVPR_WALK_HD inline
+#endif
+#endif
+
+struct ConvDiv {
+    unsigned long long mul;
+    int shift;
+};
+
+HVPR_WALK_HD ConvDiv conv_div_make(int d) {
+    int l = 0;
+    while ((1ll << l) < (long long)d) ++l;
+    ConvDiv c;
+    c.shift = 31 + l;
+    c.mul = (1ull << c.shift) / (unsigned long long)d + 1ull;
+    return c;
+}
+
+HVPR_WALK_HD int conv_div(int r, ConvDiv c) { return (int)(((unsigned long long)(unsigned)r * c.mul) >> c.shift); }
+
+HVPR_WALK_HD int conv_walk_step(int it, int n_ct, int &ct) {
+    const int xcd = it & 7, j = it >> 3;
+    ct = j % n_ct;
+    return (j / n_ct) * 8 + xcd;
+}
+
+constexpr unsigned long long CONV_TAB_HOLE = 1ull << 31;
+
+HVPR_WALK_HD unsigned long long conv_run_entry(int run, int n_runs, int run_px, int hw, int ct) {
+    if (run >= n_runs) return CONV_TAB_HOLE;
+    const long long m0 = (long long)run * run_px;
+    const unsigned n = (unsigned)(m0 / hw), rem = (unsigned)(m0 % hw);
+    return (unsigned long long)rem | (unsigned long long)((unsigned)ct | n << 12) << 32;
+}
+
+struct ConvRunPixel {
+    int n, oy, ox;
+};
+
+HVPR_WALK_HD ConvRunPixel conv_run_pixel(int n0, int rem0, int j, int hw, int ow, ConvDiv by_hw, ConvDiv by_ow) {
+    const int p = rem0 + j;
+    const int dn = conv_div(p, by_hw);
+    const int r = p - dn * hw;
+    ConvRunPixel px;
+    px.n = n0 + dn;
+    px.oy = conv_div(r, by_ow);
+    px.ox = r - px.oy * ow;
+    return px;
+}
diff --git a/hvpr_amd/kernels.py b/hvpr_amd/kernels.py
--- a/hvpr_amd/kernels.py
+++ b/hvpr_amd/kernels.py
@@ -430,7 +430,10 @@
 
 
 def _tile_channels(tile_cfg):
-    return 128 if tile_cfg == 0 else 64
+    return {0: 128, 3: 32}.get(tile_cfg, 64)
+
+
+HEAD_TILE_MAX_COLUMNS = 96
 
 
 def pack_conv(weight, scale=None, shift=None, stride=1, relu=True, tile_cfg=0):
@@ -473,6 +476,9 @@
         if isinstance(pc, PackedConvWino):
             shape = (N, H, W, pc.cout, pc.px_groups)
             size, build = lib().hvpr_conv2d_wino_tab_bytes, lib().hvpr_conv2d_wino_tab_build
+        elif pc.taps == 1:
+            shape = (N, H, W, pc.cout_pad, pc.tile_cfg)
+            size, build = lib().hvpr_conv2d_run_tab_bytes, lib().hvpr_conv2d_run_tab_build
         else:
             shape = (N, H, W, pc.taps, pc.stride, pc.cout_pad, pc.tile_cfg)
             size, build = lib().hvpr_conv2d_tab_bytes, lib().hvpr_conv2d_tab_build
@@ -573,6 +579,14 @@
         out = torch.empty((N, OH * pc.up, OW * pc.up, pc.cout), dtype=torch.float32, device=x.device)
     assert out.shape[:3] == (N, OH * pc.up, OW * pc.up) and out.is_contiguous()
     tab = _walk_table(pc, N, H, W, x.device) if use_table else 0
+    if pc.taps == 1:
+        assert pc.stride == 1, "a 1x1 convolution has stride 1"
+        check(lib().hvpr_conv2d_run_nhwc_f32(_ptr(x, torch.float32, "conv input"), N, H, W, cin, pc.w.data_ptr(), pc.bias.data_ptr(),
+                                             pc.cout, pc.cout_pad, pc.up, 1 if pc.relu else 0, _ptr(gate, torch.float32, "gate"),
+                                             _ptr(resid, torch.float32, "resid"), 0 if resid is None else resid.shape[-1],
+                                             out.data_ptr(), out.shape[-1], int(out_coff), pc.tile_cfg, tab, _stream()),
+              "hvpr_conv2d_run_nhwc_f32")
+        return out
     check(lib().hvpr_conv2d_nhwc_tab_f32(_ptr(x, torch.float32, "conv input"), N, H, W, cin, pc.w.data_ptr(),
                                          pc.bias.data_ptr(), pc.taps, pc.stride, pc.cout, pc.cout_pad, pc.up,
                                          1 if pc.relu else 0, _ptr(gate, torch.float32, "gate"),
diff --git a/include/hvpr_amd.h b/include/hvpr_amd.h
--- a/include/hvpr_amd.h
+++ b/include/hvpr_amd.h
@@ -93,6 +93,11 @@
                              int taps, int stride, int cout, int cout_pad, int up, int relu, const float *gate,
                              const float *resid, int resid_cstride, float *out, int out_cstride, int out_coff,
                              int tile_cfg, const void *table, hvpr_stream_t stream);
+size_t hvpr_conv2d_run_tab_bytes(int N, int H, int W, int cout_pad, int tile_cfg);
+int hvpr_conv2d_run_tab_build(int N, int H, int W, int cout_pad, int tile_cfg, void *table, hvpr_stream_t stream);
+int hvpr_conv2d_run_nhwc_f32(const float *in, int N, int H, int W, int Cin, const float *w_packed, const float *bias, int cout,
+                             int cout_pad, int up, int relu, const float *gate, const float *resid, int resid_cstride, float *out,
+                             int out_cstride, int out_coff, int tile_cfg, const void *table, hvpr_stream_t stream);
 
 int hvpr_spatial_gate_f32(const float *y, int N, int H, int W, int C, const float *w18, float conv_bias, float bn_scale,
                           float bn_shift, float *gate, hvpr_stream_t stream);
```

Result: no change. 466.8 frames/s (median of 6 runs) (+0.8%).
